# Ecogenomics/CheckM

Hardware: AMD Instinct MI355X
Metric: bins/hour (lineage_wf-equiv marker path: tree pass + analyze pass + qa, from genes.faa files) + residues*HMMs/s (higher is better)
Workload: dtype f16/i16 (SSV/MSV bytes held exactly, Viterbi words) + f32 (Forward/Backward)

## Files before the change

checkm_amd/csrc/cascade_dev.h:

```cpp
#pragma once
#include <hip/hip_runtime.h>
#include "dev_types.h"

namespace ckm {

constexpr float LOG2E_F = 1.44269504088896341f, LN2_F = 0.69314718055994529f;

__device__ __forceinline__ uint32_t queue_len(const WorkQueue &q) { return min(*q.count, q.cap); }

__device__ __forceinline__ float approx_ln(float x) { return __log2f(x) * LN2_F; }

__device__ __forceinline__ bool ws_alloc(const CascadeDev &cd, unsigned long long n, unsigned long long &off) {
  n = (n + 31ull) & ~31ull;
  off = atomicAdd(cd.ws_top, n);
  if (off + n > cd.ws_cap) { atomicOr(&cd.gcnt[CC_STATUS], (uint32_t)CS_WS); return false; }
  return true;
}

__device__ __forceinline__ bool ws2_alloc(const CascadeDev &cd, unsigned long long n, unsigned long long &off) {
  n = (n + 31ull) & ~31ull;
  const unsigned long long at = atomicAdd(cd.ws2_top, n);
  if (at + n > cd.ws2_cap) return false;
  off = cd.ws2_base + at;
  return true;
}

__device__ __forceinline__ void queue_push(const CascadeDev &cd, uint32_t *lists, int counter, int cls, uint32_t cap, uint32_t value, uint32_t overflow_bit) {
  const uint32_t pos = atomicAdd(&cd.cnt[counter + cls], 1u);
  if (pos < cap) lists[(size_t)cls * cap + pos] = value; else atomicOr(&cd.gcnt[CC_STATUS], overflow_bit);
}

__device__ __forceinline__ void pass_to_forward(const CascadeDev &cd, const DevModel &md, uint32_t pi, uint32_t model, uint32_t seq) {
  const int L = cd.seq_len[seq];
  unsigned long long off;
  if (!ws_alloc(cd, (unsigned long long)(L + 1) * 6ull, off)) return;
  const uint32_t t = atomicAdd(&cd.gcnt[CC_FWORK], 1u);
  if (t >= cd.cap_fwork) { atomicOr(&cd.gcnt[CC_STATUS], (uint32_t)CS_FWORK); return; }
  FbWork w;
  w.model = model; w.seq = seq; w.i0 = 0; w.Ld = L; w.Lcfg = L; w.multihit = 1;
  w.xs_off = off; w.aux_off = 0; w.mxf_off = 0; w.mxb_off = 0; w.path_off = 0;
  w.slot = t; w.full = 0; w.cand = pi; w.pass = 0xffffffffu;
  cd.fwork[t] = w;
  queue_push(cd, cd.fq, CC_FQ, md.fb_cls, cd.cap_fq, t, (uint32_t)CS_FWORK);
}

}
```

checkm_amd/csrc/cascade_regions.h:

```cpp
#pragma once
#include <hip/hip_runtime.h>
#include "dev_types.h"
#include "cascade_dev.h"
#include "xlane.h"

namespace ckm {

#ifndef CKM_LD2
#define CKM_LD2(p) __hip_atomic_load((p), __ATOMIC_RELAXED, __HIP_MEMORY_SCOPE_AGENT)
#endif

constexpr float RT1_F = 0.25f, RT2_F = 0.10f, RT3_F = 0.20f;
constexpr int ENS_CAP0 = 16;

__device__ __forceinline__ unsigned long long al32(unsigned long long v) { return (v + 31ull) & ~31ull; }

__device__ __forceinline__ void emit_region(const CascadeDev &cd, const DevModel &md, const FbWork &pw, int L, int ri, int rj, bool multi) {
  const uint32_t rid = atomicAdd(&cd.gcnt[CC_REG], 1u);
  if (rid >= cd.cap_reg) { atomicOr(&cd.gcnt[CC_STATUS], (uint32_t)CS_REG); return; }
  RegionRec rec; rec.pass = pw.pass; rec.i = ri; rec.j = rj; rec.multi = multi ? 1 : 0; rec.target = 0xffffffffu; rec.pad = 0;
  const unsigned long long Mp = (unsigned long long)md.fbQ * 64ull, Ld = (unsigned long long)(rj - ri + 1);
  unsigned long long off;
  if (!multi) {
    unsigned long long pos = 0;
    const unsigned long long xs = pos; pos = al32(pos + (Ld + 1) * 6);
    const unsigned long long aux = pos; pos = al32(al32(pos + (Ld + 1) * 3) + (Ld + 1) * 5);
    const unsigned long long mf = pos; pos = al32(pos + (Ld + 1) * 3 * Mp);
    unsigned long long mb = mf;
    if (!cd.env_inplace) { mb = pos; pos = al32(pos + (Ld + 1) * 2 * Mp); }
    if (!ws2_alloc(cd, pos, off)) rec.target = REGION_DEFERRED;
    else {
      const uint32_t e = atomicAdd(&cd.gcnt[CC_EWORK], 1u);
      if (e < cd.cap_ework) {
        FbWork w;
        w.model = pw.model; w.seq = pw.seq; w.i0 = ri - 1; w.Ld = (int32_t)Ld; w.Lcfg = L; w.multihit = 0;
        w.xs_off = off + xs; w.aux_off = off + aux; w.mxf_off = off + mf; w.mxb_off = off + mb; w.path_off = 0;
        w.slot = e; w.full = 1; w.cand = pw.cand; w.pass = pw.pass;
        cd.ework[e] = w;
        queue_push(cd, cd.eq, CC_EQ, md.fb_cls, cd.cap_eq, e, (uint32_t)CS_EWORK);
        rec.target = e;
      } else atomicOr(&cd.gcnt[CC_STATUS], (uint32_t)CS_EWORK);
    }
  } else {
    const unsigned long long cap = Ld < (unsigned long long)ENS_CAP0 ? Ld : (unsigned long long)ENS_CAP0;
    unsigned long long pos = 0;
    const unsigned long long nseg = pos; pos += 256;
    const unsigned long long seg = pos; pos += (unsigned long long)ENS_NSAMPLES * cap * 4;
    const unsigned long long n2 = pos; pos = al32(pos + Ld);
    const unsigned long long nres = pos;
    const unsigned long long xs = pos; pos = al32(pos + (Ld + 1) * 6);
    const unsigned long long mx = pos; pos = al32(pos + (Ld + 1) * 4 * Mp);
    const unsigned long long code = pos; pos = al32(pos + ((unsigned long long)ENS_NSAMPLES * (Ld + 1) + 1) / 2);
    const unsigned long long ratio = pos; pos = al32(pos + (unsigned long long)ENS_NSAMPLES * (Ld + 1));
    if (!ws2_alloc(cd, pos, off)) rec.target = REGION_DEFERRED;
    else {
      const uint32_t r = atomicAdd(&cd.gcnt[CC_RWORK], 1u);
      if (r < cd.cap_rwork) {
        EnsWork e;
        e.model = pw.model; e.seq = pw.seq; e.i0 = ri - 1; e.Ld = (int32_t)Ld; e.Lcfg = L; e.cap = (int32_t)cap;
        e.xs_off = off + xs; e.mx_off = off + mx; e.code_off = off + code; e.ratio_off = off + ratio;
        e.seg_off = off + seg; e.nseg_off = off + nseg; e.n2_off = off + n2;
        const unsigned long long hoff = atomicAdd(cd.hens_top, nres);
        e.host_off = (hoff + nres <= cd.hens_cap) ? hoff : ~0ull;
        if (e.host_off == ~0ull) atomicOr(&cd.gcnt[CC_STATUS], (uint32_t)CS_RWORK);
        rec.pad = (e.host_off == ~0ull) ? 0xffffffffu : (uint32_t)hoff;
        cd.ens[r] = e;
        FbWork w;
        w.model = pw.model; w.seq = pw.seq; w.i0 = ri - 1; w.Ld = (int32_t)Ld; w.Lcfg = L; w.multihit = 1;
        w.xs_off = e.xs_off; w.aux_off = 0; w.mxf_off = e.mx_off; w.mxb_off = 0; w.path_off = 0;
        w.slot = r; w.full = 2; w.cand = pw.cand; w.pass = pw.pass;
        cd.rwork[r] = w;
        queue_push(cd, cd.rq, CC_RQ, md.fb_cls, cd.cap_rq, r, (uint32_t)CS_RWORK);
        if (cd.ensq) { const uint32_t k = atomicAdd(cd.ensq_cnt, 1u); if (k < cd.cap_rwork) cd.ensq[k] = r; }
        rec.target = r;
      } else atomicOr(&cd.gcnt[CC_STATUS], (uint32_t)CS_RWORK);
    }
  }
  cd.h_reg[rid] = rec;
}

template <bool XL>
__device__ __forceinline__ void region_scan(const CascadeDev &cd, const DevModel &md, const FbWork &w, float *__restrict__ ws, int lane) {
  const int L = w.Ld;
  float *aux = ws + w.aux_off;
  float btp = 0.f, etp = 0.f;
  int ri = -1; bool trig = false;
  for (int base = 1; base <= L; base += 64) {
    const int row = base + lane;
    const bool ok = row <= L;
    const float bt = ok ? (XL ? CKM_LD2(&aux[(size_t)row * 3]) : aux[(size_t)row * 3]) : 0.f, et = ok ? (XL ? CKM_LD2(&aux[(size_t)row * 3 + 1]) : aux[(size_t)row * 3 + 1]) : 0.f,
                nj = ok ? (XL ? CKM_LD2(&aux[(size_t)row * 3 + 2]) : aux[(size_t)row * 3 + 2]) : 0.f;
    const int nrow = min(64, L - base + 1);
    const float btp0 = btp, etp0 = etp;
    float pb = 0.f, pe = 0.f;
    for (int r = 0; r < nrow; ++r) {
      btp = btp + read_lane(bt, r); etp = etp + read_lane(et, r);
      if (lane == r) { pb = btp; pe = etp; }
    }
    if (ok) { aux[(size_t)row * 3] = pb; aux[(size_t)row * 3 + 1] = pe; }
    __threadfence();
    __builtin_amdgcn_wave_barrier();
    float pbm = btp0, pem = etp0;
    for (int r = 0; r < nrow; ++r) {
      const float btn = read_lane(pb, r), etn = read_lane(pe, r), mo = 1.0f - read_lane(nj, r);
      const int j = base + r;
      if (!trig) {
        if (mo - (btn - pbm) < RT2_F) ri = j; else if (ri == -1) ri = j;
        if (mo >= RT1_F) trig = true;
      } else if (mo - (etn - pem) < RT2_F) {
        const float e0 = (ri - 1 >= 1) ? CKM_LD2(&aux[(size_t)(ri - 1) * 3 + 1]) : 0.f;
        float mx = -1.0f;
        for (int z = ri + lane; z <= j; z += 64) {
          const float bz = (z - 1 >= 1) ? CKM_LD2(&aux[(size_t)(z - 1) * 3]) : 0.f;
          const float a = CKM_LD2(&aux[(size_t)z * 3 + 1]) - e0, b = btn - bz;
          const float en = a < b ? a : b;
          if (en > mx) mx = en;
        }
        mx = wave_max(mx);
        if (lane == 0) emit_region(cd, md, w, L, ri, j, mx >= RT3_F);
        ri = -1; trig = false;
      }
      pbm = btn; pem = etn;
    }
  }
}

}
```

checkm_amd/csrc/ckm_api.hip:

```cpp
#include "ckm_host.h"

namespace ckm {
static thread_local std::string g_err;
void set_last_error(const std::string &m) { g_err = m; }

}

std::atomic<uint64_t> g_uid{1};

const std::string &ckm_seq_name(const ckm_seqs *s, uint32_t i) { return s->names.at(i); }
int ckm_ctx_device(const ckm_ctx *ctx) { return ctx->device; }
void ckm_ctx_parallel_for(ckm_ctx *ctx, size_t n, size_t chunk, const std::function<void(size_t, size_t)> &f) {
  if (ctx->w[0].pool) ctx->w[0].pool->run(n, chunk, f); else if (n) f(0, n);
}
void *ckm_ctx_reduce_scratch(ckm_ctx *ctx, size_t bytes) { ctx->reduce_scratch.ensure(bytes); return ctx->reduce_scratch.p; }

extern "C" const char *ckm_last_error(void) { return g_err.c_str(); }
extern "C" int ckm_abi_version(void) { return CKM_ABI_VERSION; }

extern "C" int ckm_device_count(int *n) {
  return guarded([&] {
    if (!n) throw Error(CKM_EINVAL, "n is NULL");
    int c = 0;
    hipError_t e = hipGetDeviceCount(&c);
    if (e != hipSuccess) { *n = 0; throw Error(CKM_ENODEV, std::string("hipGetDeviceCount: ") + hipGetErrorString(e)); }
    *n = c;
  });
}

extern "C" int ckm_ctx_create(int device, ckm_ctx **out) {
  setenv("GPU_MAX_HW_QUEUES", "16", 0);
  return guarded([&] {
    if (!out) throw Error(CKM_EINVAL, "out is NULL");
    *out = nullptr;
    int c = 0;
    if (hipGetDeviceCount(&c) != hipSuccess || c <= 0) throw Error(CKM_ENODEV, "no HIP device visible: libcheckm_hip has no CPU path");
    if (device < 0 || device >= c) throw Error(CKM_ENODEV, "device index out of range");
    HIPCHK(hipSetDevice(device));
    hipDeviceProp_t prop;
    HIPCHK(hipGetDeviceProperties(&prop, device));
    if (std::string(prop.gcnArchName).compare(0, 6, "gfx950") != 0)
      throw Error(CKM_ENODEV, std::string("device is ") + prop.gcnArchName + "; this library carries gfx950 code objects only");
    std::unique_ptr<ckm_ctx> ctx(new ckm_ctx());
    ctx->device = device;
    memset(&ctx->stats, 0, sizeof(ctx->stats));
    if (const char *e = getenv("CKM_WORKERS")) ctx->nclasses = std::max(1, std::min(NWORKERS, atoi(e)));
    ctx->nworkers = ctx->nclasses * ctx->ngroups;
    const int hw = (int)std::thread::hardware_concurrency();
    int host_threads = std::max(1, std::min(hw, std::max(8, std::min(16, hw / 8))));
    if (const char *e = getenv("CKM_HOST_THREADS")) host_threads = std::max(1, std::min(64, atoi(e)));
    size_t fre = 0, tot = 0;
    size_t budget = (size_t)8 << 30;
    if (hipMemGetInfo(&fre, &tot) == hipSuccess) budget = std::min<size_t>((size_t)96 << 30, fre / 4) / ctx->nworkers;
    if (const char *e = getenv("CKM_WS_BUDGET_MB")) budget = std::max<size_t>(16, strtoull(e, nullptr, 10)) << 20;
    const bool pooled = ctx->nworkers == 1;
    const int nside = choose_side_streams(ctx->nworkers);
    const int slot = pooled ? pool_next_slot(device) : 0;
    for (auto &w : ctx->w) {
      w.device = device; w.id = (int)(&w - ctx->w);
      if (&w - ctx->w >= ctx->nworkers) continue;
      if (pooled) pool_assign_streams(w, device, slot);
      else {
        w.own_streams = true;
        HIPCHK(hipStreamCreateWithFlags(&w.stream, hipStreamNonBlocking));
        w.nside = nside;
        w.nss = nside >= 8 ? 4 : std::max(1, nside / 3); w.nch = nside - w.nss;
        for (int k = 0; k < 16; ++k) {
          if (k >= nside) { w.side[k] = w.side[k % nside]; continue; }
          HIPCHK(hipStreamCreateWithFlags(&w.side[k], hipStreamNonBlocking));
        }
        HIPCHK(hipStreamCreateWithFlags(&w.ens_stream, hipStreamNonBlocking));
      }
      {
        int lo = 0, hi = 0;
        HIPCHK(hipDeviceGetStreamPriorityRange(&lo, &hi));
        HIPCHK(hipStreamCreateWithPriority(&w.late[0], hipStreamNonBlocking, hi));
        for (int k = 1; k < 4; ++k) w.late[k] = w.late[0];
      }
      for (auto &e : w.ev) HIPCHK(hipEventCreate(&e));
      for (auto &e : w.cev) HIPCHK(hipEventCreateWithFlags(&e, hipEventDisableTiming));
      for (auto &e : w.cls_ev) HIPCHK(hipEventCreateWithFlags(&e, hipEventDisableTiming));
      for (auto &e : w.grp_ev) HIPCHK(hipEventCreateWithFlags(&e, hipEventDisableTiming));
      for (auto &e : w.ens_ev) HIPCHK(hipEventCreateWithFlags(&e, hipEventDisableTiming));
      memset(&w.stats, 0, sizeof(w.stats));
      w.ws_budget = budget;
      if (!(getenv("CKM_WS_VMM") && atoi(getenv("CKM_WS_VMM")) == 0)) { w.ws.vmm = true; w.ws.va_bytes = budget + ((size_t)8 << 30); }
      if (const char *e = getenv("CKM_WS_PER_CELL")) w.caps.ws_per_cell = (float)atof(e);
      w.pool.reset(new HostPool(host_threads));
    }
    *out = ctx.release();
  });
}

extern "C" int ckm_ctx_reserve(ckm_ctx *ctx, uint64_t pairs, double cells) {
  return guarded([&] {
    if (!ctx) throw Error(CKM_EINVAL, "ctx is NULL");
    ctx->settle();
    Worker &w = ctx->w[0];
    const uint64_t est = (uint64_t)(1.05 * cells * (double)w.caps.ws_per_cell + (double)pairs * 24.0) + ((uint64_t)256 << 20);
    const size_t want = (size_t)std::min<uint64_t>(std::max<uint64_t>(est, (uint64_t)1 << 30), (uint64_t)w.ws_budget);
    if (w.ws.cap >= want) return;
    const int device = ctx->device;
    std::lock_guard<std::mutex> lock(ctx->reserve_mutex);
    ctx->reserve_thread = std::thread([&w, want, device] {
      if (hipSetDevice(device) != hipSuccess) return;
      try { w.ws.ensure(want); } catch (...) {  }
    });
  });
}

extern "C" void ckm_ctx_destroy(ckm_ctx *ctx) {
  if (!ctx) return;
  ctx->settle();
  (void)hipSetDevice(ctx->device);
  (void)hipDeviceSynchronize();
  for (auto &w : ctx->w) {
    if (!w.stream) continue;
    for (auto &e : w.ev) (void)hipEventDestroy(e);
    for (auto &e : w.cev) if (e) (void)hipEventDestroy(e);
    for (auto &e : w.cls_ev) if (e) (void)hipEventDestroy(e);
    for (auto &e : w.grp_ev) if (e) (void)hipEventDestroy(e);
    for (auto &e : w.ens_ev) if (e) (void)hipEventDestroy(e);
    if (w.late[0]) (void)hipStreamDestroy(w.late[0]);
    if (!w.own_streams) continue;
    for (int k = 0; k < w.nside; ++k) (void)hipStreamDestroy(w.side[k]);
    if (w.ens_stream) (void)hipStreamDestroy(w.ens_stream);
    (void)hipStreamDestroy(w.stream);
  }
  const int device = ctx->device;
  delete ctx;
  dev_cache_trim(device);
}

namespace {
struct Arena {
  std::vector<uint8_t> host;
  template <class T> size_t add(const std::vector<T> &v) {
    const size_t off = (host.size() + 255) & ~(size_t)255;
    host.resize(off + std::max<size_t>(16, v.size() * sizeof(T)));
    if (!v.empty()) memcpy(host.data() + off, v.data(), v.size() * sizeof(T));
    return off;
  }
};
}

extern "C" int ckm_profiles_load(ckm_ctx *ctx, const char *hmm_path, ckm_profiles **out) {
  return guarded([&] {
    if (!ctx || !hmm_path || !out) throw Error(CKM_EINVAL, "NULL argument");
    *out = nullptr;
    HIPCHK(hipSetDevice(ctx->device));
    std::unique_ptr<ckm_profiles> p(new ckm_profiles());
    p->ctx = ctx;
    p->hmm = read_hmm_file(hmm_path);
    const size_t n = p->hmm.size();
    p->prof.resize(n);
    p->too_long.assign(n, 0);
    {
      std::vector<std::unique_ptr<Error>> errs(n);
      auto one = [&](size_t lo, size_t hi) {
        for (size_t i = lo; i < hi; ++i) {
          try { p->prof[i] = configure_profile(p->hmm[i]); }
          catch (const Error &e) {
            if (e.code == CKM_ERANGE) { p->too_long[i] = 1; p->prof[i] = HostProfile(); p->prof[i].M = p->hmm[i].M; p->prof[i].ssvQ = p->prof[i].fbQ = p->prof[i].vitQH = 1; }
            else errs[i].reset(new Error(e));
          }
        }
      };
      if (ctx->w[0].pool && n > 8) ctx->w[0].pool->run(n, 4, one); else one(0, n);
      for (size_t i = 0; i < n; ++i) if (errs[i]) throw Error(*errs[i]);
    }
    Arena ar;
    struct Off { size_t ssv, ssvh, rbv, vit_e, vit_t, rf, ftr, v16e, v16t, ssv8; };
    std::vector<Off> off(n);
    for (size_t i = 0; i < n; ++i) {
      const HostProfile &hp = p->prof[i];
      off[i] = Off{ar.add(hp.ssv_tbl), ar.add(hp.ssv_tbl_h), ar.add(hp.rbv), ar.add(hp.vit_e), ar.add(hp.vit_t), ar.add(hp.rf), ar.add(hp.ftr), ar.add(hp.vit16_e), ar.add(hp.vit16_t), ar.add(hp.ssv8_tbl_h)};
    }
    std::unique_ptr<DevBuf> tables(new DevBuf());
    tables->ensure(std::max<size_t>(256, ar.host.size()));
    HIPCHK(hipMemcpy(tables->p, ar.host.data(), ar.host.size(), hipMemcpyHostToDevice));
    const uint8_t *base = tables->as<uint8_t>();
    p->tables.push_back(std::move(tables));
    for (size_t i = 0; i < n; ++i) {
      const HostHMM &h = p->hmm[i];
      const HostProfile &hp = p->prof[i];
      DevModel d;
      memset(&d, 0, sizeof(d));
      d.M = hp.M; d.ssvQ = hp.ssvQ; d.fbQ = hp.fbQ; d.vitQH = hp.vitQH;
      d.fb_cls = fb_class_id(hp.fbQ); d.vitx_cls = vit_class_id(hp.vitQH); d.vit16Q = hp.vit16Q;
      d.vit_cls = hp.vit16Q ? vit16_class_id(hp.vit16Q) : d.vitx_cls;
      if (!p->too_long[i] && (d.fb_cls < 0 || d.vit_cls < 0)) throw Error(CKM_ERANGE, "model " + h.name + " is longer than the instantiated kernel classes (DESIGN.md limits)");
      d.base_b = hp.base_b; d.bias_b = hp.bias_b; d.tbm_b = hp.tbm_b; d.tec_b = hp.tec_b; d.scale_b = hp.scale_b;
      d.scale_w = hp.scale_w; d.base_w = hp.base_w; d.wE_loop = hp.wE_loop; d.wE_move = hp.wE_move;
      d.fE_loop = hp.fE_loop; d.fE_move = hp.fE_move;
      d.bt00 = hp.bt00; d.bt01 = hp.bt01; d.bt10 = hp.bt10; d.bt11 = hp.bt11; d.bpi0 = hp.bpi0; d.bpi1 = hp.bpi1;
      for (int x = 0; x < NROWS; ++x) d.beo1[x] = hp.beo1[x];
      d.thr_msv_f1 = hp.thr_msv_f1; d.thr_msv_f1_nat = hp.thr_msv_f1_nat; d.thr_msv_f2 = hp.thr_msv_f2; d.thr_vit_f2 = hp.thr_vit_f2; d.thr_fwd_f3 = hp.thr_fwd_f3;
      d.ssv_tbl = reinterpret_cast<const int16_t *>(base + off[i].ssv); d.ssv_tbl_h = reinterpret_cast<const uint16_t *>(base + off[i].ssvh);
      d.rbv = base + off[i].rbv; d.vit_e = reinterpret_cast<const uint32_t *>(base + off[i].vit_e);
      d.vit_t = reinterpret_cast<const uint32_t *>(base + off[i].vit_t); d.rf = reinterpret_cast<const float *>(base + off[i].rf);
      d.ftr = reinterpret_cast<const float *>(base + off[i].ftr);
      d.ssv8_tbl_h = hp.ssv8Q ? reinterpret_cast<const uint16_t *>(base + off[i].ssv8) : nullptr;
      d.vit16_e = reinterpret_cast<const uint32_t *>(base + off[i].v16e); d.vit16_t = reinterpret_cast<const uint32_t *>(base + off[i].v16t);
      p->dm.push_back(d);
      if (!p->too_long[i]) p->maxMp = std::max(p->maxMp, hp.fbQ * NL);
    }
    p->d_models.ensure(p->dm.size() * sizeof(DevModel));
    HIPCHK(hipMemcpy(p->d_models.p, p->dm.data(), p->dm.size() * sizeof(DevModel), hipMemcpyHostToDevice));
    *out = p.release();
  });
}

extern "C" int ckm_profiles_count(const ckm_profiles *p, int32_t *n) {
  if (!p || !n) { set_last_error("NULL argument"); return CKM_EINVAL; }
  *n = (int32_t)p->hmm.size();
  return CKM_OK;
}

extern "C" int ckm_profiles_header(const ckm_profiles *p, int32_t i, ckm_model_header *o) {
  if (!p || !o || i < 0 || i >= (int32_t)p->hmm.size()) { set_last_error("bad argument"); return CKM_EINVAL; }
  const HostHMM &h = p->hmm[i];
  o->name = h.name.c_str(); o->acc = h.has_acc ? h.acc.c_str() : nullptr; o->desc = h.has_desc ? h.desc.c_str() : nullptr;
  o->leng = h.M; o->has_ga = h.has_ga; o->has_tc = h.has_tc; o->has_nc = h.has_nc;
  for (int k = 0; k < 2; ++k) { o->ga[k] = h.ga[k]; o->tc[k] = h.tc[k]; o->nc[k] = h.nc[k]; }
  for (int k = 0; k < 6; ++k) o->evparam[k] = h.evparam[k];
  o->searchable = p->too_long[(size_t)i] ? 0 : 1;
  return CKM_OK;
}

extern "C" void ckm_profiles_free(ckm_profiles *p) {
  if (!p) return;
  if (p->ctx) (void)hipSetDevice(p->ctx->device);
  delete p;
}

static void build_lentab(ckm_seqs *s) {
  HostProfile dummy;
  dummy.scale_b = (float)(3.0 / 0.69314718055994529);
  dummy.scale_w = (float)(500.0 / 0.69314718055994529);
  s->lentab.resize((size_t)s->maxL + 1);
  for (int L = 0; L <= s->maxL; ++L) {
    const LenCfg m = len_config(dummy, L, true), u = len_config(dummy, L, false);
    LenEntry e;
    e.loop_m = m.loop; e.move_m = m.move; e.loop_u = u.loop; e.move_u = u.move;
    e.nullsc = m.nullsc; e.bias_tail = m.bias_tail; e.w_move = m.w_move; e.tjb_b = m.tjb_b;
    s->lentab[L] = e;
  }
}

static SeqColumns seq_columns(ckm_seqs *s) {
  return SeqColumns{&s->bin_off, &s->seq_bin, &s->order, &s->order_off, &s->len, &s->off, &s->bin_res, &s->dsq, &s->names, &s->descs, &s->total_res, &s->maxL};
}

static void finish_seqs(ckm_seqs *s) {
  const uint32_t nseq = s->nseq;
  build_seq_order(ingest_threads(), seq_columns(s));
  build_lentab(s);
  hipStream_t up = s->ctx->w[0].late[3];
  trace_pt(&s->ctx->w[0], "seqs: tables built");
  s->d_res.ensure(s->dsq.size() + 16); s->d_off.ensure((size_t)nseq * 8 + 16); s->d_len.ensure((size_t)nseq * 4 + 16);
  s->d_order.ensure(s->order.size() * 4 + 16); s->d_lentab.ensure(s->lentab.size() * sizeof(LenEntry) + 16);
  trace_pt(&s->ctx->w[0], "seqs: device buffers allocated");
  {
    std::lock_guard<std::mutex> lock(s->ctx->upload_mutex);
    struct Part { DevBuf *d; const void *src; size_t bytes; };
    const Part parts[5] = {{&s->d_res, s->dsq.data(), s->dsq.size()}, {&s->d_off, s->off.data(), (size_t)nseq * 8}, {&s->d_len, s->len.data(), (size_t)nseq * 4},
                           {&s->d_order, s->order.data(), s->order.size() * 4}, {&s->d_lentab, s->lentab.data(), s->lentab.size() * sizeof(LenEntry)}};
    size_t tot = 0;
    for (auto &pt : parts) tot += (pt.bytes + 255) & ~(size_t)255;
    s->ctx->upload.begin(tot);
    for (auto &pt : parts) s->ctx->upload.put(up, pt.d->p, pt.src, pt.bytes);
    HIPCHK(hipStreamSynchronize(up));
  }
  trace_pt(&s->ctx->w[0], "seqs: uploaded");
// ... 259 lines not shown
```

checkm_amd/csrc/ckm_debug.hip:

```cpp
#include "ckm_host.h"

extern "C" int ckm_debug_stages(ckm_ctx *ctx_, const ckm_profiles *p, const ckm_seqs *s, const uint32_t *model, const uint32_t *seq,
                                uint32_t npairs, ckm_stage_scores *out) {
  return guarded([&] {
    if (!ctx_ || !p || !s || !model || !seq || !out) throw Error(CKM_EINVAL, "NULL argument");
    for (uint32_t j = 0; j < npairs; ++j) if (model[j] < p->hmm.size() && p->too_long[model[j]]) throw Error(CKM_ERANGE, "model longer than the instantiated kernel classes");
    ctx_->settle();
    Worker *ctx = &ctx_->w[0];
    ctx->plan_key.clear();
    HIPCHK(hipSetDevice(ctx->device));
    const DevModel *dm = p->d_models.as<DevModel>();
    const LenEntry *lt = s->d_lentab.as<LenEntry>();
    const uint8_t *res = s->d_res.as<uint8_t>();
    const uint64_t *off = s->d_off.as<uint64_t>();
    const int32_t *dlen = s->d_len.as<int32_t>();
    memset(out, 0, sizeof(*out) * npairs);
    std::vector<SsvBlockWork> work(npairs); std::vector<uint32_t> ids(seq, seq + npairs);
    std::map<int, std::vector<uint32_t>> byQ;
    for (uint32_t i = 0; i < npairs; ++i) {
      if (model[i] >= p->hmm.size() || seq[i] >= s->nseq) throw Error(CKM_EINVAL, "pair index out of range");
      work[i].model = model[i]; work[i].list_start = i; work[i].count = 1; work[i].pair_start = i; byQ[ssv_class(p->prof[model[i]])].push_back(i);
    }
    std::vector<SsvBlockWork> sorted; std::vector<std::pair<int, std::pair<size_t, size_t>>> groups;
    for (auto &kv : byQ) { groups.push_back({kv.first, {sorted.size(), kv.second.size()}}); for (uint32_t i : kv.second) sorted.push_back(work[i]); }
// ... 50 lines not shown
    std::vector<int32_t> vx(npairs); std::vector<float> vs(npairs);
    HIPCHK(hipMemcpyAsync(vx.data(), ctx->vitx.p, npairs * 4, hipMemcpyDeviceToHost, ctx->stream));
    HIPCHK(hipMemcpyAsync(vs.data(), ctx->vits.p, npairs * 4, hipMemcpyDeviceToHost, ctx->stream));
    HIPCHK(hipStreamSynchronize(ctx->stream));
    FbBatch fb; uint64_t pos = 0;
    for (uint32_t i = 0; i < npairs; ++i) {
      const int L = s->len[seq[i]];
      FbWork w; memset(&w, 0, sizeof(w));
      w.model = model[i]; w.seq = seq[i]; w.i0 = 0; w.Ld = L; w.Lcfg = L; w.multihit = 1; w.full = 0; w.slot = i;
      w.xs_off = pos; pos += ((uint64_t)(L + 1) * 6 + 31) & ~(uint64_t)31;
      w.aux_off = pos; pos += ((uint64_t)(L + 1) * 3 + 31) & ~(uint64_t)31;
      fb.work.push_back(w);
    }
    ctx->ws.ensure(pos * 4 + 256);
    run_fb(ctx, p, s, fb, true, false, false, nullptr);
    EventIndex ei; ei.build(fb.events, npairs);
    for (uint32_t i = 0; i < npairs; ++i) {
      const int L = s->len[seq[i]];
      const LenEntry &le = s->lentab[L];
      ckm_stage_scores &o = out[i];
      o.ssv_maxv = maxv[i]; o.msv_xJ = xJ[i]; o.msv_sc = usc[i]; o.null_sc = le.nullsc;
      o.msvp_xJ = xJp[i]; o.msvp_sc = uscp[i];
      const float p1 = (float)L / (float)(L + 1);
      const float nullsc = (float)(log((double)raw[(size_t)i * 3]) + (double)raw[(size_t)i * 3 + 1] * kLn2);
      o.bias_sc = nullsc + (float)L * logf(p1) + logf(1.0f - p1);
      o.vit_xC = vx[i]; o.vit_sc = vs[i];
      o.fwd_xC = fb.fout[i].xC; o.fwd_nscale = fb.fout[i].nscale;
      o.fwd_sc = finish_forward(fb.fout[i].xC, le.move_m, ei.scales(i));
    }
  });
}

extern "C" int ckm_debug_ssv(ckm_ctx *ctx_, const ckm_profiles *p, const ckm_seqs *s, uint32_t model, const uint32_t *seq, uint32_t n,
                             uint32_t per_block, int32_t lanes, uint16_t *smax, uint8_t *route, float *usc, int32_t *info) {
  return guarded([&] {
    if (!ctx_ || !p || !s || !seq || !smax || !route || !usc) throw Error(CKM_EINVAL, "NULL argument");
    if (model >= p->hmm.size()) throw Error(CKM_EINVAL, "model index out of range");
    if (p->too_long[model]) throw Error(CKM_ERANGE, "model longer than the instantiated kernel classes");
    if (n == 0 || n > (1u << 24)) throw Error(CKM_EINVAL, "between 1 and 2^24 sequences");
    if (lanes != 0 && lanes != 8 && lanes != 16) throw Error(CKM_EINVAL, "lanes must be 0, 8 or 16");
    std::vector<int64_t> pos_of(s->nseq, -1);
    for (uint32_t i = 0; i < n; ++i) {
      if (seq[i] >= s->nseq) throw Error(CKM_EINVAL, "sequence index out of range");
      if (s->len[seq[i]] <= 0) throw Error(CKM_EINVAL, "empty sequence (the lists of a search hold none)");
      if (pos_of[seq[i]] >= 0) throw Error(CKM_EINVAL, "sequence listed twice");
      pos_of[seq[i]] = i;
    }
    const HostProfile &hp = p->prof[model];
    int cls = ssv_class(hp);
    if (lanes == 8) { if (!hp.ssv8Q) throw Error(CKM_ERANGE, "the model has no 8-lane SSV image"); cls = 100 + hp.ssv8Q; }
    if (lanes == 16) { if (hp.ssvQ > 64) throw Error(CKM_ERANGE, "the model has no 16-lane SSV image"); cls = hp.ssvQ; }
    const uint32_t pb = per_block ? per_block : ssv_per_block(cls);
    const int threads = ssv_threads_for(cls);
    std::vector<SsvBlockWork> work;
    for (uint32_t a = 0; a < n; a += pb) { SsvBlockWork w; w.model = model; w.list_start = a; w.count = std::min(pb, n - a); w.pair_start = a; work.push_back(w); }
    if (info) { info[0] = cls; info[1] = threads; info[2] = (int32_t)pb; info[3] = (int32_t)work.size(); }
    ctx_->settle();
    Worker *ctx = &ctx_->w[0];
    ctx->plan_key.clear();
    HIPCHK(hipSetDevice(ctx->device));
    const DevModel *dm = p->d_models.as<DevModel>();
    const LenEntry *lt = s->d_lentab.as<LenEntry>();
    const uint8_t *res = s->d_res.as<uint8_t>();
    const uint64_t *off = s->d_off.as<uint64_t>();
    const int32_t *dlen = s->d_len.as<int32_t>();
    ctx->work.ensure(work.size() * sizeof(SsvBlockWork)); ctx->idx.ensure((size_t)n * 4); ctx->maxv.ensure((size_t)n * 2 + 64);
    ctx->surv.ensure((size_t)n * sizeof(PairRec)); ctx->nores.ensure((size_t)n * sizeof(PairRec)); ctx->counters.ensure(64);
    wcopy(ctx, ctx->work.p, work.data(), work.size() * sizeof(SsvBlockWork), hipMemcpyHostToDevice);
    wcopy(ctx, ctx->idx.p, seq, (size_t)n * 4, hipMemcpyHostToDevice);
    HIPCHK(hipMemsetAsync(ctx->maxv.p, 0xff, (size_t)n * 2, ctx->stream));
    HIPCHK(hipMemsetAsync(ctx->counters.p, 0, 64, ctx->stream));
    SsvEpi epi; memset(&epi, 0, sizeof(epi));
    epi.lentab = lt; epi.maxv = ctx->maxv.as<uint16_t>();
    if (launch_ssv(cls, (int)work.size(), threads, ctx->stream, ctx->work.as<SsvBlockWork>(), dm, res, off, dlen, ctx->idx.as<uint32_t>(), epi))
      throw Error(CKM_ERANGE, "no SSV kernel instance");
    const SsvEpi fin{lt, ctx->surv.as<PairRec>(), ctx->counters.as<uint32_t>(), n, ctx->nores.as<PairRec>(), ctx->counters.as<uint32_t>() + 1, n, nullptr};
    if (launch_ssv(cls, (int)work.size(), threads, ctx->stream, ctx->work.as<SsvBlockWork>(), dm, res, off, dlen, ctx->idx.as<uint32_t>(), fin))
      throw Error(CKM_ERANGE, "no SSV kernel instance");
    HIPCHK(hipGetLastError());
    uint32_t cnt[2] = {0, 0};
    HIPCHK(hipMemcpyAsync(smax, ctx->maxv.p, (size_t)n * 2, hipMemcpyDeviceToHost, ctx->stream));
    HIPCHK(hipMemcpyAsync(cnt, ctx->counters.p, 8, hipMemcpyDeviceToHost, ctx->stream));
    HIPCHK(hipStreamSynchronize(ctx->stream));
    if (cnt[0] > n || cnt[1] > n) throw Error(CKM_EHIP, "the SSV finish appended " + std::to_string(cnt[0]) + " survivors and " + std::to_string(cnt[1]) + " exact-kernel pairs for " + std::to_string(n) + " pairs");
    std::vector<PairRec> sv(cnt[0]), nr(cnt[1]);
    if (cnt[0]) wcopy(ctx, sv.data(), ctx->surv.p, (size_t)cnt[0] * sizeof(PairRec), hipMemcpyDeviceToHost);
    if (cnt[1]) wcopy(ctx, nr.data(), ctx->nores.p, (size_t)cnt[1] * sizeof(PairRec), hipMemcpyDeviceToHost);
    for (uint32_t i = 0; i < n; ++i) {
      if (smax[i] == 0xffffu) throw Error(CKM_EHIP, "the SSV kernel wrote no Smax for list entry " + std::to_string(i));
      route[i] = 0; usc[i] = 0.f;
    }
    auto place = [&](const PairRec &r, uint8_t code) {
      if (r.model != model || r.seq >= s->nseq || pos_of[r.seq] < 0) throw Error(CKM_EHIP, "the SSV finish reported a pair that was not listed: model " + std::to_string(r.model) + ", sequence " + std::to_string(r.seq));
      const size_t i = (size_t)pos_of[r.seq];
      if (route[i] != 0) throw Error(CKM_EHIP, "the SSV finish reported list entry " + std::to_string(i) + " twice");
      route[i] = code; usc[i] = r.usc;
    };
    for (const PairRec &r : sv) place(r, 1);
    for (const PairRec &r : nr) place(r, 2);
  });
}

extern "C" int ckm_debug_filters(ckm_ctx *ctx_, const ckm_profiles *p, const ckm_seqs *s, const uint32_t *model, const uint32_t *seq,
                                 const float *usc, const float *filtersc, uint32_t n, int32_t mode, uint32_t nblocks,
                                 ckm_filter_result *out, uint32_t *status) {
  return guarded([&] {
    if (!ctx_ || !p || !s || !model || !seq || !usc || !out || !status) throw Error(CKM_EINVAL, "NULL argument");
    if (mode < CKM_FILTERS_VIT16 || mode > CKM_FILTERS_CHAIN) throw Error(CKM_EINVAL, "unknown mode");
    if (mode != CKM_FILTERS_CHAIN && !filtersc) throw Error(CKM_EINVAL, "NULL argument");
    if (n == 0 || n > (1u << 22)) throw Error(CKM_EINVAL, "between 1 and 2^22 pairs");
    if (nblocks > 65536) throw Error(CKM_EINVAL, "at most 65536 workgroups");
    const uint32_t nb = nblocks ? nblocks : GRID_VIT;
    bool present[NVC] = {false};
    std::vector<std::vector<uint32_t>> vq(NVC);
    unsigned long long ws_need = 0;
    int q16 = -1;
    for (uint32_t i = 0; i < n; ++i) {
      if (model[i] >= p->hmm.size() || seq[i] >= s->nseq) throw Error(CKM_EINVAL, "pair index out of range");
      if (p->too_long[model[i]]) throw Error(CKM_ERANGE, "model longer than the instantiated kernel classes");
      if (s->len[seq[i]] <= 0) throw Error(CKM_EINVAL, "empty sequence (the lists of a search hold none)");
      const DevModel &d = p->dm[model[i]];
      if (mode == CKM_FILTERS_VIT16) {
        if (!d.vit16Q) throw Error(CKM_ERANGE, "the model has no 16-lane Viterbi image");
        if (q16 >= 0 && q16 != d.vit16Q) throw Error(CKM_EINVAL, "the pairs of a VIT16 call must share one 16-lane class");
        q16 = d.vit16Q;
      }
      const int c = (mode == CKM_FILTERS_VIT16 || mode == CKM_FILTERS_CHAIN) ? d.vit_cls : d.vitx_cls;
      if (c < 0 || c >= NVC || d.vitx_cls < NV16 || d.vitx_cls >= NVC || d.fb_cls < 0 || d.fb_cls >= NFC) throw Error(CKM_ERANGE, "no kernel instance for this model length");
      present[c] = true; present[d.vitx_cls] = true;
      if (mode != CKM_FILTERS_CHAIN) vq[c].push_back(i);
      ws_need += (((unsigned long long)(s->len[seq[i]] + 1) * 6ull) + 31ull) & ~31ull;
    }
    ctx_->settle();
    Worker *ctx = &ctx_->w[0];
    ctx->plan_key.clear();
    HIPCHK(hipSetDevice(ctx->device));
    const DevModel *dm = p->d_models.as<DevModel>();
    const LenEntry *lt = s->d_lentab.as<LenEntry>();
    const uint8_t *res = s->d_res.as<uint8_t>();
    const uint64_t *off = s->d_off.as<uint64_t>();
    const int32_t *dlen = s->d_len.as<int32_t>();
    hipStream_t st = ctx->stream;
    auto table = [](DevBuf &b, size_t bytes) { b.ensure(std::max<size_t>(64, bytes)); return b.p; };
    uint32_t *d_cnt = (uint32_t *)table(ctx->c_cnt, 2 * CC_SIZE * 4);
    unsigned long long *d_tops = (unsigned long long *)table(ctx->c_tops, 4 * 8);
    CascadeDev cd; memset(&cd, 0, sizeof(cd));
    cd.cand = (PairRec *)table(ctx->c_cand, (size_t)n * sizeof(PairRec)); cd.cap_cand = n;
    cd.bias_raw = (float *)table(ctx->c_bias, (size_t)n * 8);
    cd.vit_fast = (float *)table(ctx->c_vfast, (size_t)n * 4); cd.vit_exact = (float *)table(ctx->c_vexact, (size_t)n * 4);
    cd.vit_flag = (uint32_t *)table(ctx->c_vflag, (size_t)n * 4); cd.route = (uint8_t *)table(ctx->c_route, n);
    cd.vq = (uint32_t *)table(ctx->c_vq, (size_t)n * NVC * 4); cd.vxq = (uint32_t *)table(ctx->c_vxq, (size_t)n * NVC * 4); cd.cap_vq = n;
    cd.fq = (uint32_t *)table(ctx->c_fq, (size_t)n * NFC * 4); cd.cap_fq = n;
    cd.fwork = (FbWork *)table(ctx->c_fwork, (size_t)n * sizeof(FbWork)); cd.cap_fwork = n;
    cd.gcnt = d_cnt; cd.cnt = d_cnt + CC_SIZE;
    cd.ws_top = d_tops; cd.ws_cap = 2 * ws_need;
    cd.seq_len = dlen;
    cd.margin_msv = kMarginMsv; cd.margin_vit = kMarginVit; cd.margin_fwd = kMarginFwd;
    int32_t *d_xC = (int32_t *)table(ctx->vitx, (size_t)n * 4); float *d_sc = (float *)table(ctx->vits, (size_t)n * 4); uint32_t *d_flag = (uint32_t *)table(ctx->vitf, (size_t)n * 4);
    std::vector<PairRec> pr(n);
    for (uint32_t i = 0; i < n; ++i) { pr[i].model = model[i]; pr[i].seq = seq[i]; pr[i].usc = usc[i]; pr[i].filtersc = mode == CKM_FILTERS_CHAIN ? 0.f : filtersc[i]; }
    std::vector<uint32_t> cnt(2 * CC_SIZE, 0u);
    cnt[CC_SIZE + CC_CAND] = n;
    wcopy(ctx, cd.cand, pr.data(), (size_t)n * sizeof(PairRec), hipMemcpyHostToDevice);
    for (int c = 0; c < NVC; ++c) if (!vq[c].empty()) {
      cnt[CC_SIZE + CC_VQ + c] = (uint32_t)vq[c].size();
      wcopy(ctx, cd.vq + (size_t)c * n, vq[c].data(), vq[c].size() * 4, hipMemcpyHostToDevice);
    }
    wcopy(ctx, d_cnt, cnt.data(), cnt.size() * 4, hipMemcpyHostToDevice);
    HIPCHK(hipMemsetAsync(d_tops, 0, 4 * 8, st));
    auto sentinels = [&] {
      HIPCHK(hipMemsetAsync(cd.vit_fast, 0xff, (size_t)n * 4, st)); HIPCHK(hipMemsetAsync(cd.vit_exact, 0xff, (size_t)n * 4, st));
      HIPCHK(hipMemsetAsync(cd.vit_flag, 0xff, (size_t)n * 4, st));
    };
    sentinels();
    HIPCHK(hipMemsetAsync(cd.bias_raw, 0xff, (size_t)n * 8, st));
    HIPCHK(hipMemsetAsync(cd.route, mode == CKM_FILTERS_CHAIN ? 0xee : 1, n, st));
    HIPCHK(hipMemsetAsync(d_xC, 0xff, (size_t)n * 4, st)); HIPCHK(hipMemsetAsync(d_sc, 0xff, (size_t)n * 4, st)); HIPCHK(hipMemsetAsync(d_flag, 0xff, (size_t)n * 4, st));
    uint32_t *gc = cd.cnt;
    int rc = 0;
    auto exact_launches = [&] {
      for (int c = NVC - 1; c >= NV16; --c) if (present[c])
        rc |= launch_vit(kVitQH[c - NV16], std::max(64u, GRID_VIT / 4), st, WorkQueue{cd.vxq + (size_t)c * cd.cap_vq, gc + CC_VXQ + c, cd.cap_vq}, cd.cand, dm, lt, res, off, dlen, nullptr, nullptr, nullptr, false, &cd);
    };
    if (mode == CKM_FILTERS_CHAIN) {
      launch_bias_filter(st, GRID_MSV, cd, dm, lt, res, off);
      sentinels();
    }
    if (mode == CKM_FILTERS_WAVE_FAST_PLAIN) {
      for (int c = NVC - 1; c >= NV16; --c) if (present[c])
        rc |= launch_vit(kVitQH[c - NV16], nb, st, WorkQueue{cd.vq + (size_t)c * cd.cap_vq, gc + CC_VQ + c, cd.cap_vq}, cd.cand, dm, lt, res, off, dlen, d_xC, d_sc, d_flag, true, nullptr);
    } else {
      for (int c = NVC - 1; c >= 0; --c) if (present[c]) {
        const WorkQueue qv{cd.vq + (size_t)c * cd.cap_vq, gc + CC_VQ + c, cd.cap_vq};
        if (c < NV16) rc |= launch_vit16(kVit16Q[c], nb, st, qv, cd.cand, dm, lt, res, off, dlen, cd);
        else rc |= launch_vit(kVitQH[c - NV16], nb, st, qv, cd.cand, dm, lt, res, off, dlen, nullptr, nullptr, nullptr, true, &cd);
      }
      exact_launches();
    }
    if (rc) throw Error(CKM_ERANGE, "no Viterbi kernel instance");
    HIPCHK(hipGetLastError());
    std::vector<float> raw((size_t)n * 2), vfast(n), vexact(n), psc(n);
    std::vector<uint32_t> vflag(n), pflag(n), lists_vq((size_t)n * NVC), lists_vxq((size_t)n * NVC);
    std::vector<int32_t> pxC(n); std::vector<uint8_t> route(n);
    HIPCHK(hipMemcpyAsync(cnt.data(), d_cnt, cnt.size() * 4, hipMemcpyDeviceToHost, st));
    HIPCHK(hipMemcpyAsync(pr.data(), cd.cand, (size_t)n * sizeof(PairRec), hipMemcpyDeviceToHost, st));
    HIPCHK(hipMemcpyAsync(raw.data(), cd.bias_raw, (size_t)n * 8, hipMemcpyDeviceToHost, st));
    HIPCHK(hipMemcpyAsync(vfast.data(), cd.vit_fast, (size_t)n * 4, hipMemcpyDeviceToHost, st));
    HIPCHK(hipMemcpyAsync(vexact.data(), cd.vit_exact, (size_t)n * 4, hipMemcpyDeviceToHost, st));
    HIPCHK(hipMemcpyAsync(vflag.data(), cd.vit_flag, (size_t)n * 4, hipMemcpyDeviceToHost, st));
    HIPCHK(hipMemcpyAsync(route.data(), cd.route, n, hipMemcpyDeviceToHost, st));
    HIPCHK(hipMemcpyAsync(lists_vq.data(), cd.vq, (size_t)n * NVC * 4, hipMemcpyDeviceToHost, st));
    HIPCHK(hipMemcpyAsync(lists_vxq.data(), cd.vxq, (size_t)n * NVC * 4, hipMemcpyDeviceToHost, st));
    HIPCHK(hipMemcpyAsync(pxC.data(), d_xC, (size_t)n * 4, hipMemcpyDeviceToHost, st));
    HIPCHK(hipMemcpyAsync(psc.data(), d_sc, (size_t)n * 4, hipMemcpyDeviceToHost, st));
    HIPCHK(hipMemcpyAsync(pflag.data(), d_flag, (size_t)n * 4, hipMemcpyDeviceToHost, st));
    HIPCHK(hipStreamSynchronize(st));
    *status = cnt[CC_STATUS];
    const uint32_t nfw = std::min(cnt[CC_FWORK], n);
    std::vector<FbWork> fw(nfw);
    if (nfw) wcopy(ctx, fw.data(), cd.fwork, (size_t)nfw * sizeof(FbWork), hipMemcpyDeviceToHost);
    auto bits_of = [](float f) { uint32_t u; memcpy(&u, &f, 4); return u; };
    auto name = [&](uint32_t i) { return "pair " + std::to_string(i) + " (model " + std::to_string(model[i]) + ", sequence " + std::to_string(seq[i]) + ", L = " + std::to_string(s->len[seq[i]]) + ")"; };
    const bool plain = mode == CKM_FILTERS_WAVE_FAST_PLAIN;
    for (uint32_t i = 0; i < n; ++i) {
      ckm_filter_result &o = out[i];
      o.bias_d = raw[2 * (size_t)i]; o.bias_e = raw[2 * (size_t)i + 1]; o.filtersc = pr[i].filtersc;
      o.vit_fast = plain ? psc[i] : vfast[i]; o.vit_exact = vexact[i]; o.vit_flag = plain ? pflag[i] : vflag[i];
      o.vit_xC = plain ? pxC[i] : INT32_MAX; o.route = route[i]; o.n_vq = o.n_vxq = o.n_fwork = 0;
      if (pr[i].model != model[i] || pr[i].seq != seq[i]) throw Error(CKM_EHIP, "the candidate record of " + name(i) + " was overwritten");
    }
    if (cnt[CC_SIZE + CC_CAND] != n) throw Error(CKM_EHIP, "the candidate counter changed");
    for (int c = 0; c < NVC; ++c) {
      const uint32_t nv = cnt[CC_SIZE + CC_VQ + c], nx = cnt[CC_SIZE + CC_VXQ + c];
      if (nv > n || nx > n) throw Error(CKM_EHIP, "queue of class " + std::to_string(c) + " holds " + std::to_string(nv) + " FAST and " + std::to_string(nx) + " exact entries for " + std::to_string(n) + " pairs");
      if ((nv || nx) && !present[c]) throw Error(CKM_EHIP, "entries in the queue of class " + std::to_string(c) + ", which no pair of the call has");
      for (uint32_t k = 0; k < nv; ++k) {
        const uint32_t i = lists_vq[(size_t)c * n + k];
        if (i >= n) throw Error(CKM_EHIP, "FAST queue of class " + std::to_string(c) + ", position " + std::to_string(k) + ": " + std::to_string(i) + " is no pair of the call");
        if (p->dm[model[i]].vit_cls != c && !(mode != CKM_FILTERS_CHAIN && p->dm[model[i]].vitx_cls == c)) throw Error(CKM_EHIP, name(i) + " sits in the FAST queue of class " + std::to_string(c));
        if (out[i].n_vq++) throw Error(CKM_EHIP, name(i) + " sits twice in the FAST queue of class " + std::to_string(c));
        if (bits_of(out[i].vit_fast) == 0xffffffffu || out[i].vit_flag == 0xffffffffu) throw Error(CKM_EHIP, "FAST queue of class " + std::to_string(c) + ", position " + std::to_string(k) + ": the kernel wrote nothing for " + name(i));
      }
      for (uint32_t k = 0; k < nx; ++k) {
        const uint32_t i = lists_vxq[(size_t)c * n + k];
        if (i >= n) throw Error(CKM_EHIP, "exact queue of class " + std::to_string(c) + ", position " + std::to_string(k) + ": " + std::to_string(i) + " is no pair of the call");
        if (p->dm[model[i]].vitx_cls != c) throw Error(CKM_EHIP, name(i) + " sits in the exact queue of class " + std::to_string(c));
        if (out[i].n_vxq++) throw Error(CKM_EHIP, name(i) + " sits twice in the exact queue of class " + std::to_string(c));
        if (bits_of(out[i].vit_exact) == 0xffffffffu) throw Error(CKM_EHIP, "exact queue of class " + std::to_string(c) + ", position " + std::to_string(k) + ": the kernel wrote nothing for " + name(i));
      }
    }
    if (cnt[CC_FWORK] > n) throw Error(CKM_EHIP, std::to_string(cnt[CC_FWORK]) + " Forward items for " + std::to_string(n) + " pairs");
    for (uint32_t t = 0; t < nfw; ++t) {
      const uint32_t i = fw[t].cand;
      if (i >= n || fw[t].model != model[i] || fw[t].seq != seq[i]) throw Error(CKM_EHIP, "Forward item " + std::to_string(t) + " is no pair of the call");
      if (out[i].n_fwork++) throw Error(CKM_EHIP, name(i) + " was handed to Forward twice");
    }
    if (mode == CKM_FILTERS_CHAIN) for (uint32_t i = 0; i < n; ++i) {
      if (out[i].route == 0xee || bits_of(out[i].bias_d) == 0xffffffffu) throw Error(CKM_EHIP, "the bias filter wrote nothing for " + name(i));
    }
  });
}

extern "C" int ckm_debug_envelopes(ckm_ctx *ctx_, const ckm_profiles *p, const ckm_seqs *s, const uint32_t *model, const uint32_t *seq,
                                   const int32_t *ienv, const int32_t *jenv, uint32_t n, ckm_envelope_result *out) {
  return guarded([&] {
    if (!ctx_ || !p || !s || !model || !seq || !ienv || !jenv || !out) throw Error(CKM_EINVAL, "NULL argument");
    ctx_->settle();
    Worker *ctx = &ctx_->w[0];
    HIPCHK(hipSetDevice(ctx->device));
    std::vector<EnvReq> req(n); std::vector<EnvRes> res;
    for (uint32_t i = 0; i < n; ++i) {
      if (model[i] >= p->hmm.size() || seq[i] >= s->nseq || ienv[i] < 1 || jenv[i] > s->len[seq[i]] || jenv[i] < ienv[i]) throw Error(CKM_EINVAL, "bad envelope");
      req[i] = {model[i], seq[i], ienv[i], jenv[i]};
    }
    rescore_envelopes(ctx, p, s, req, res);
    for (uint32_t i = 0; i < n; ++i) {
      out[i].envsc = res[i].envsc; out[i].oasc = res[i].oasc; out[i].fwd_xC = res[i].xC; out[i].nscale = res[i].nscale; out[i].ok = res[i].ok;
      for (int x = 0; x < 20; ++x) out[i].null2[x] = res[i].null2[x];
      out[i].hmm_from = res[i].hmm_from; out[i].hmm_to = res[i].hmm_to; out[i].ali_from = res[i].ali_from; out[i].ali_to = res[i].ali_to;
    }
  });
}

extern "C" int ckm_debug_region(ckm_ctx *ctx_, const ckm_profiles *p, const ckm_seqs *s, uint32_t model, uint32_t seq, int32_t ireg, int32_t jreg,
                                float *n2sum, int32_t *segs, int32_t *nseg, int32_t cap, int32_t *env, int32_t envcap, int32_t *nenv) {
  return guarded([&] {
    if (!ctx_ || !p || !s || !n2sum || !segs || !nseg || !env || !nenv) throw Error(CKM_EINVAL, "NULL argument");
    if (model >= p->hmm.size() || seq >= s->nseq || ireg < 1 || jreg > s->len[seq] || jreg < ireg) throw Error(CKM_EINVAL, "bad region");
    ctx_->settle();
    Worker *ctx = &ctx_->w[0];
    HIPCHK(hipSetDevice(ctx->device));
    std::vector<RegionReq> req{{model, seq, ireg, jreg}}; std::vector<RegionRes> res;
    run_ensembles(ctx, p, s, req, res);
    const RegionRes &r = res[0];
    for (size_t i = 0; i < r.n2sum.size(); ++i) n2sum[i] = r.n2sum[i];
    for (int t = 0; t < ENS_NSAMPLES; ++t) {
      if (r.nseg[t] > cap) throw Error(CKM_ERANGE, "segment table too small");
      nseg[t] = r.nseg[t];
      for (int d = 0; d < r.nseg[t]; ++d) { const Seg &g = r.segs[(size_t)t * r.cap + d]; int32_t *o = segs + ((size_t)t * cap + d) * 4; o[0] = g.sqfrom; o[1] = g.sqto; o[2] = g.hmmfrom; o[3] = g.hmmto; }
    }
    if ((int)r.env.size() > envcap) throw Error(CKM_ERANGE, "envelope table too small");
    *nenv = (int32_t)r.env.size();
    for (size_t e = 0; e < r.env.size(); ++e) { env[e * 4] = r.env[e].sqfrom; env[e * 4 + 1] = r.env[e].sqto; env[e * 4 + 2] = r.env[e].hmmfrom; env[e * 4 + 3] = r.env[e].hmmto; }
  });
}
```

checkm_amd/csrc/ckm_host.h:

```cpp
#pragma once
#include <hip/hip_runtime.h>
#include <algorithm>
#include <array>
#include <atomic>
#include <chrono>
#include <cmath>
#include <condition_variable>
#include <cstring>
#include <exception>
#include <functional>
#include <map>
#include <memory>
#include <mutex>
#include <numeric>
#include <thread>
#include "ckm_internal.h"
#include "dev_types.h"
#include "host_pool.h"
#include "stream_plan.h"

namespace ckm {

int launch_ssv(int Q, int nblocks, int threads, hipStream_t stream, const SsvBlockWork *work, const DevModel *models,
               const uint8_t *res, const uint64_t *seq_off, const int32_t *seq_len, const uint32_t *lists, const SsvEpi &epi );
void launch_msv_full(hipStream_t stream, uint32_t nblocks, WorkQueue queue, const PairRec *pairs, const DevModel *models, const LenEntry *lentab,
                     const uint8_t *res, const uint64_t *seq_off, const int32_t *seq_len, int32_t *out_xJ, float *out_usc, int maxMp,
                     const CascadeDev *cd );
void launch_bias(hipStream_t stream, PairRec *pairs, uint32_t npairs, const DevModel *models, const LenEntry *lentab,
                 const uint8_t *res, const uint64_t *seq_off, const int32_t *seq_len, float *raw);
int launch_msv16(int Q, uint32_t nblocks, hipStream_t stream, WorkQueue queue, const PairRec *pairs, const DevModel *models, const LenEntry *lentab,
                 const uint8_t *res, const uint64_t *seq_off, const int32_t *seq_len, const CascadeDev &cd, int32_t *out_xJ = nullptr , float *out_usc = nullptr);
int launch_vit16(int Q, uint32_t nblocks, hipStream_t stream, WorkQueue queue, const PairRec *pairs, const DevModel *models, const LenEntry *lentab,
                 const uint8_t *res, const uint64_t *seq_off, const int32_t *seq_len, const CascadeDev &cd);
int launch_vit(int QH, uint32_t nblocks, hipStream_t stream, WorkQueue queue, const PairRec *pairs, const DevModel *models,
               const LenEntry *lentab, const uint8_t *res, const uint64_t *seq_off, const int32_t *seq_len, int32_t *out_xC, float *out_sc,
               uint32_t *out_flag, bool fast, const CascadeDev *cd );
int launch_fwd(int Q, uint32_t nblocks, hipStream_t stream, WorkQueue queue, FbWork *work, const DevModel *models,
               const LenEntry *lentab, const uint8_t *res, const uint64_t *seq_off, float *ws, FwdOut *out,
               ScaleEvent *events, uint32_t *nevents, uint32_t cap_events, const CascadeDev *cd );
int launch_bwd(int Q, uint32_t nblocks, hipStream_t stream, WorkQueue queue, const FbWork *work, const DevModel *models,
               const LenEntry *lentab, const uint8_t *res, const uint64_t *seq_off, float *ws, const FwdOut *fout, int32_t *range_err);
int launch_oa(int Q, uint32_t nblocks, hipStream_t stream, WorkQueue queue, const FbWork *work, const DevModel *models,
              float *ws, const int32_t *range_err, const FwdOut *fout, EnvOut *out);

void launch_ensemble(hipStream_t stream, const EnsWork *work, const uint32_t *list , const uint32_t *count, uint32_t cap, uint32_t grid_regions, int max_Mp,
                     const DevModel *models, const LenEntry *lentab, const uint8_t *res, const uint64_t *seq_off, float *ws, const uint32_t *seeds,
                     float *host_res );
void launch_bias_filter(hipStream_t stream, uint32_t nblocks, const CascadeDev &cd, const DevModel *models, const LenEntry *lentab,
                        const uint8_t *res, const uint64_t *seq_off);
void launch_regions(hipStream_t stream, uint32_t nblocks, const uint32_t *list, const uint32_t *count, uint32_t cap, const FbWork *fwork,
                    const CascadeDev &cd, const DevModel *models, float *ws);
#define HIPCHK(expr)                                                                                         \
  do {                                                                                                       \
    hipError_t e_ = (expr);                                                                                  \
    if (e_ != hipSuccess) throw Error(CKM_EHIP, std::string(#expr) + ": " + hipGetErrorString(e_));          \
  } while (0)

struct DevCache {
  std::mutex m;
  std::multimap<size_t, void *> free_[16];
  size_t cached[16] = {0};
  static DevCache &get() { static DevCache c; return c; }
  void *take(int dev, size_t want, size_t &got) {
    std::lock_guard<std::mutex> lock(m);
    auto &f = free_[dev & 15];
    auto it = f.lower_bound(want);
    if (it != f.end() && it->first <= want + want / 2 + (1 << 20)) { void *p = it->second; got = it->first; cached[dev & 15] -= got; f.erase(it); return p; }
    return nullptr;
  }
  bool give(int dev, void *p, size_t cap) {
    if (cap >= ((size_t)2 << 30)) return false;
    std::lock_guard<std::mutex> lock(m);
    if (cached[dev & 15] + cap > ((size_t)64 << 30)) return false;
    free_[dev & 15].emplace(cap, p); cached[dev & 15] += cap;
    return true;
  }
  void trim(int dev) {
    std::multimap<size_t, void *> f;
    { std::lock_guard<std::mutex> lock(m); f.swap(free_[dev & 15]); cached[dev & 15] = 0; }
    for (auto &kv : f) (void)hipFree(kv.second);
  }
};
inline void dev_cache_trim(int dev) { DevCache::get().trim(dev); }

struct DevBuf {
  void *p = nullptr; size_t cap = 0; int dev = -1;
  bool vmm = false; size_t va_bytes = (size_t)128 << 30, chunk_bytes = 0; std::vector<hipMemGenericAllocationHandle_t> chunks;
  void drop(bool drained = false) {
    if (!p) return;
    if (!drained || dev < 0 || !DevCache::get().give(dev, p, cap)) (void)hipFree(p);
    p = nullptr; cap = 0;
  }
  void ensure(size_t bytes) {
    if (bytes <= cap) return;
    if (vmm) {
      if (p) { grow_mapped(bytes); return; }
      try { grow_mapped(bytes); return; }
      catch (const Error &) { if (p || cap) throw; vmm = false; }
    }
    drop();
    (void)hipGetDevice(&dev);
    size_t want = bytes + std::min<size_t>(bytes / 4, (size_t)1 << 30) + 256;
    size_t got = 0;
    if (void *q = DevCache::get().take(dev, want, got)) { p = q; cap = got; return; }
    hipError_t e = hipMalloc(&p, want);
    if (e != hipSuccess) {
      DevCache::get().trim(dev);
      e = hipMalloc(&p, want);
    }
    if (e != hipSuccess) { p = nullptr; throw Error(CKM_ENOMEM, "hipMalloc of " + std::to_string(want) + " bytes failed: " + hipGetErrorString(e)); }
    cap = want;
  }
  void grow_mapped(size_t bytes) {
    int dev = 0; (void)hipGetDevice(&dev);
    hipMemAllocationProp prop = {};
    prop.type = hipMemAllocationTypePinned; prop.location.type = hipMemLocationTypeDevice; prop.location.id = dev;
    auto fail = [&](const char *what, hipError_t e) { throw Error(CKM_ENOMEM, std::string(what) + " failed while growing a mapped buffer to " + std::to_string(bytes) + " bytes: " + hipGetErrorString(e)); };
    if (!p) {
      size_t gran = 0;
      hipError_t e = hipMemGetAllocationGranularity(&gran, &prop, hipMemAllocationGranularityRecommended);
      if (e != hipSuccess || !gran) fail("hipMemGetAllocationGranularity", e);
      chunk_bytes = (((size_t)1 << 30) + gran - 1) / gran * gran;
      va_bytes = (va_bytes + chunk_bytes - 1) / chunk_bytes * chunk_bytes;
      e = hipMemAddressReserve(&p, va_bytes, 0, nullptr, 0);
      if (e != hipSuccess) { p = nullptr; fail("hipMemAddressReserve", e); }
    }
    const size_t want = (bytes + 256 + chunk_bytes - 1) / chunk_bytes * chunk_bytes;
    if (want > va_bytes) throw Error(CKM_ENOMEM, "a mapped buffer cannot grow beyond its " + std::to_string(va_bytes) + " reserved bytes");
    hipMemAccessDesc acc = {}; acc.location.type = hipMemLocationTypeDevice; acc.location.id = dev; acc.flags = hipMemAccessFlagsProtReadWrite;
    while (cap < want) {
      hipMemGenericAllocationHandle_t h;
      hipError_t e = hipMemCreate(&h, chunk_bytes, &prop, 0);
      if (e != hipSuccess) { DevCache::get().trim(dev); e = hipMemCreate(&h, chunk_bytes, &prop, 0); }
      if (e != hipSuccess) fail("hipMemCreate", e);
      e = hipMemMap(static_cast<char *>(p) + cap, chunk_bytes, 0, h, 0);
      if (e != hipSuccess) { (void)hipMemRelease(h); fail("hipMemMap", e); }
      e = hipMemSetAccess(static_cast<char *>(p) + cap, chunk_bytes, &acc, 1);
      if (e != hipSuccess) { (void)hipMemUnmap(static_cast<char *>(p) + cap, chunk_bytes); (void)hipMemRelease(h); fail("hipMemSetAccess", e); }
      chunks.push_back(h); cap += chunk_bytes;
    }
  }
  template <class T> T *as() const { return reinterpret_cast<T *>(p); }
  ~DevBuf() {
    if (vmm) {
      if (p && cap) (void)hipMemUnmap(p, cap);
      for (auto h : chunks) (void)hipMemRelease(h);
      if (p) (void)hipMemAddressFree(p, va_bytes);
    } else drop(std::uncaught_exceptions() == 0);
  }
  DevBuf() = default; DevBuf(const DevBuf &) = delete; DevBuf &operator=(const DevBuf &) = delete;
};

struct PinnedBuf {
  void *p = nullptr; size_t cap = 0;
  void ensure(size_t bytes) {
    if (bytes <= cap) return;
    if (p) (void)hipHostFree(p);
    p = nullptr; cap = 0;
    const size_t want = bytes + bytes / 4 + 4096;
    if (hipHostMalloc(&p, want, hipHostMallocPortable | hipHostMallocMapped) != hipSuccess) { p = nullptr; throw Error(CKM_ENOMEM, "hipHostMalloc failed"); }
    cap = want;
  }
  template <class T> T *as() const { return reinterpret_cast<T *>(p); }
  ~PinnedBuf() { if (p) (void)hipHostFree(p); }
};


void launch_upload(hipStream_t st, void *dst, const void *src_pinned, size_t bytes);
struct Stager {
  static constexpr size_t HALF = (size_t)16 << 20;
  PinnedBuf buf; hipEvent_t ev[2] = {nullptr, nullptr}; bool busy[2] = {false, false}; int half = 0; size_t top = 0;
  void begin(size_t ) {
    if (!buf.p) { buf.ensure(2 * HALF); for (auto &e : ev) HIPCHK(hipEventCreateWithFlags(&e, hipEventDisableTiming)); }
    busy[0] = busy[1] = false; half = 0; top = 0;
  }
  void put(hipStream_t st, void *dst, const void *src, size_t bytes) {
    const uint8_t *from = static_cast<const uint8_t *>(src); uint8_t *to = static_cast<uint8_t *>(dst);
    while (bytes) {
      if (top == HALF) {
        HIPCHK(hipEventRecord(ev[half], st)); busy[half] = true;
        half ^= 1; top = 0;
        if (busy[half]) { HIPCHK(hipEventSynchronize(ev[half])); busy[half] = false; }
      }
      const size_t n = std::min(bytes, HALF - top);
      uint8_t *stage = buf.as<uint8_t>() + (size_t)half * HALF + top;
      memcpy(stage, from, n);
      launch_upload(st, to, stage, n);
      top = std::min(HALF, (top + n + 255) & ~(size_t)255);
      from += n; to += n; bytes -= n;
    }
  }
  ~Stager() { for (auto &e : ev) if (e) (void)hipEventDestroy(e); }
};

struct CallStream {
  hipStream_t st = nullptr;
  hipEvent_t ev[8] = {};
  bool own = false;
  void open(int device) {
    HIPCHK(hipSetDevice(device));
    HIPCHK(hipStreamCreateWithFlags(&st, hipStreamNonBlocking));
    own = true;
    for (auto &e : ev) HIPCHK(hipEventCreate(&e));
  }
  void borrow(hipStream_t s) {
    st = s;
    for (auto &e : ev) HIPCHK(hipEventCreate(&e));
  }
  void mark(int k) { HIPCHK(hipEventRecord(ev[k], st)); }
  float ms(int a, int b) { float t = 0.f; HIPCHK(hipEventElapsedTime(&t, ev[a], ev[b])); return t; }
  template <class F> void timed(double &acc, F &&fn) {
    mark(0);
    fn();
    mark(1);
    HIPCHK(hipEventSynchronize(ev[1]));
    acc += ms(0, 1);
  }
  ~CallStream() {
    for (auto &e : ev) if (e) (void)hipEventDestroy(e);
    if (own) { (void)hipStreamSynchronize(st); (void)hipStreamDestroy(st); }
  }
  CallStream() = default; CallStream(const CallStream &) = delete; CallStream &operator=(const CallStream &) = delete;
};

}

using namespace ckm;

extern std::atomic<uint64_t> g_uid;

struct Worker {
  int device = 0;
  int id = 0;
  hipStream_t stream = nullptr;
  hipStream_t ens_stream = nullptr;
  hipStream_t side[16];
  int nside = 0;
  int nss = 0, nch = 0;
  bool own_streams = false;
  hipEvent_t ev[8];
  ckm_search_stats stats;
  std::vector<uint64_t> plan_key;
  std::vector<std::pair<int, std::pair<size_t, size_t>>> plan_groups;
  uint64_t plan_npairs = 0, plan_nblocks = 0, plan_residue_hmm = 0, plan_cells = 0, plan_pairs = 0;
  PinnedBuf h_a, h_b, h_ens;
  DevBuf work, maxv, surv, nores, counters, cand, raw, idx, vitx, vits, vitf, fbwork, fbidx, fbmodel, ws, fout, events, rerr, envout, fullx, fullu, msvwork, msvlist, enswork, ensseeds, ws_ens, enscount, vitq;
  size_t ws_budget = (size_t)8 << 30;
  std::unique_ptr<HostPool> pool;
  struct CascadeCaps { uint32_t fwork = 0, ework = 0, rwork = 0, pass = 0, reg = 0, events_f = 0, events_e = 0, seen_rwork = 0; uint64_t hens = 0;
                       uint32_t div_cand = 12, div_nores = 48, div_fwork = 160, div_ework = 256, div_rwork = 32768;
                       uint32_t fl_cand = 4096, fl_nores = 2048, fl_fwork = 2048, fl_ework = 1024, fl_rwork = 256; float ws_per_cell = 11.f, z1_per_pair = 64.f; } caps;
  DevBuf c_cnt, c_cand, c_nores, c_bias, c_vfast, c_vexact, c_vflag, c_route, c_vq, c_vxq, c_fq, c_bq, c_eq, c_rq, c_fwork, c_ework, c_rwork, c_ens, c_ensq,
         c_fout_f, c_fout_e, c_fout_r, c_rerr_e, c_rerr_r, c_tops, c_events_r, c_pass, c_reg, c_hens, c_envout, c_events_f, c_events_e;
  PinnedBuf h_cnt, h_pass, h_reg, h_envout, h_events_f, h_events_e, h_hens, h_tops;
  hipEvent_t cev[4] = {nullptr, nullptr, nullptr, nullptr};
  hipEvent_t cls_ev[16] = {};
  bool ens_pending = false;
  hipEvent_t ens_ev[17] = {};
  PinnedBuf wstage; std::mutex wstage_mutex;
  Stager stager;
  hipStream_t late[4] = {};
  bool late_round = false;
  hipEvent_t grp_ev[192] = {};
};

constexpr int kVitQH[ckm::NVW] = {1, 2, 3, 4, 5, 6, 7, 8, 10, 12, 14, 16, 24, 32};
constexpr int kVit16Q[ckm::NV16] = {1, 2, 3, 4, 5, 6, 7, 8, 10, 12, 14, 16};
constexpr int kFbQ[ckm::NFC] = {1, 2, 3, 4, 6, 8, 12, 16, 24, 32, 48, 64};
constexpr int kSsvNone = 65;
inline int vit_class_id(int QH) { for (int i = 0; i < ckm::NVW; ++i) if (kVitQH[i] == QH) return ckm::NV16 + i; return -1; }
inline int vit16_class_id(int Q16) { for (int i = 0; i < ckm::NV16; ++i) if (kVit16Q[i] == Q16) return i; return -1; }
inline int fb_class_id(int Q) { for (int i = 0; i < ckm::NFC; ++i) if (kFbQ[i] == Q) return i; return -1; }

constexpr float kMarginMsv = 0.01f, kMarginVit = 0.01f, kMarginFwd = 0.05f;
constexpr uint32_t GRID_FB = 4096, GRID_VIT = 2048, GRID_MSV = 1024;

constexpr int NWORKERS = 8;

struct ckm_ctx {
  int device = 0;
  int nworkers = 1;
  int nclasses = 1, ngroups = 1;
  DevBuf reduce_scratch;
  Worker w[NWORKERS];
  ckm_search_stats stats;
  std::mutex ssv_mutex;
  std::condition_variable ssv_cv; int ssv_turn = 0;
  std::mutex upload_mutex; Stager upload;
  std::thread reserve_thread;
  std::string reserve_error;
  std::mutex reserve_mutex;
  void settle() { std::lock_guard<std::mutex> lock(reserve_mutex); if (reserve_thread.joinable()) reserve_thread.join(); }
  std::atomic<uint64_t> fallbacks{0};
  hipEvent_t ssv_prev_done = nullptr;
};

struct ckm_profiles {
  ckm_ctx *ctx = nullptr;
  uint64_t uid = g_uid++;
  std::vector<HostHMM> hmm;
  std::vector<HostProfile> prof;
  std::vector<DevModel> dm;
  DevBuf d_models;
  std::vector<std::unique_ptr<DevBuf>> tables;
  std::vector<uint8_t> too_long;
  int maxMp = 0;
};


struct ckm_seqs {
  ckm_ctx *ctx = nullptr;
  uint64_t uid = 0;
  uint32_t nseq = 0, nbins = 0;
  std::vector<uint32_t> bin_off, seq_bin;
  std::vector<int32_t> len;
  std::vector<uint64_t> off;
  std::vector<uint8_t> dsq;
  std::vector<std::string> names, descs;
  std::vector<LenEntry> lentab;
  DevBuf d_res, d_off, d_len, d_lentab;
  uint64_t total_res = 0;
  int maxL = 0;
  std::vector<uint32_t> order, order_off;
  std::vector<uint64_t> bin_res;
  DevBuf d_order;
};

struct ckm_hits {
  std::vector<uint64_t> bin_row_off;
  std::vector<uint32_t> seq, model;
  std::vector<int32_t> tlen, qlen, dom_idx, ndom, hmm_from, hmm_to, ali_from, ali_to, env_from, env_to;
  std::vector<double> full_evalue, c_evalue, i_evalue;
  std::vector<float> full_score, full_bias, dom_score, dom_bias, acc;
  uint32_t nbins = 0;
};

static inline void drain_after_error(int code) {
  if (code != CKM_EINVAL && code != CKM_ENODEV) (void)hipDeviceSynchronize();
}
template <class F>
static inline int guarded(F &&f) {
  try { f(); return CKM_OK; }
  catch (const Error &e) { set_last_error(e.what()); drain_after_error(e.code); return e.code; }
  catch (const std::bad_alloc &) { set_last_error("out of host memory"); drain_after_error(CKM_ENOMEM); return CKM_ENOMEM; }
  catch (const std::exception &e) { set_last_error(e.what()); return CKM_EINVAL; }
}

namespace ckm {

constexpr double kLn2 = 0.69314718055994529;
constexpr double kLog2R = 1.44269504088896341;
constexpr float kOmega = 1.0f / 256.0f;
constexpr float RT1 = 0.25f, RT2 = 0.10f, RT3 = 0.20f;

struct Domain {
  int ienv, jenv; float envsc, oasc, domcorrection; int hmm_from, hmm_to, ali_from, ali_to;
  float dombias, bitscore; double lnP; bool reported;
};
struct Hit {
  uint32_t model, seq; int L; float pre_score, score; double lnP; std::vector<Domain> dom; int nreported;
};
struct Cand {
  PairRec r; float fwdsc; float fwd_xC; uint32_t slot; bool alive;
};

struct EventIndex {
  std::vector<uint32_t> first;
  std::vector<std::pair<int, float>> ev;
  void build(const ScaleEvent *e, size_t n, size_t nslots) {
    first.assign(nslots + 1, 0);
    for (size_t k = 0; k < n; ++k) if (e[k].slot < nslots) first[e[k].slot + 1]++;
    for (size_t k = 0; k < nslots; ++k) first[k + 1] += first[k];
    ev.resize(first[nslots]);
    std::vector<uint32_t> at(first.begin(), first.end() - 1);
    for (size_t k = 0; k < n; ++k) if (e[k].slot < nslots) ev[at[e[k].slot]++] = {e[k].row, e[k].scale};
    for (size_t k = 0; k < nslots; ++k) if (first[k + 1] - first[k] > 1) std::sort(ev.begin() + first[k], ev.begin() + first[k + 1]);
  }
  void build(const std::vector<ScaleEvent> &v, size_t nslots) { build(v.data(), v.size(), nslots); }
  std::vector<float> scales(uint32_t slot) const { std::vector<float> r; for (uint32_t k = first[slot]; k < first[slot + 1]; ++k) r.push_back(ev[k].second); return r; }
};

struct FbBatch {
  std::vector<FbWork> work;
  std::vector<FwdOut> fout;
  std::vector<ScaleEvent> events;
  std::vector<int32_t> rerr;
  std::vector<EnvOut> envout;
};

struct EnvReq { uint32_t model, seq; int ienv, jenv; };

struct EnvRes { bool ok; float envsc, oasc, xC; int nscale; float null2[KP]; int hmm_from, hmm_to, ali_from, ali_to; };

struct Seg { int32_t sqfrom, sqto, hmmfrom, hmmto; };

struct RegionReq { uint32_t model, seq; int ireg, jreg; };

struct RegionRes {
  std::vector<float> n2sum;
  std::vector<Seg> segs;
  std::vector<int32_t> nseg;
  int cap = 0;
  std::vector<Seg> env;
};

void pool_run(Worker *w, size_t n, size_t chunk, const std::function<void(size_t, size_t)> &f);
void wcopy(Worker *w, void *dst, const void *src, size_t bytes, hipMemcpyKind kind);
double now_ms();
float bits(float sc, float nullsc);
float finish_forward(float xC, float move, const std::vector<float> &scales);
int ssv_threads_for(int Q);
int ssv_class(const HostProfile &hp);
uint32_t ssv_per_block(int cls);
int choose_side_streams(int nworkers);
int hw_queue_budget();
void pool_assign_streams(Worker &w, int device, int slot);
// ... 31 lines not shown
```

checkm_amd/csrc/ckm_search.hip:

```cpp
#include "ckm_host.h"

namespace {

#define CKM_TRACE_PT(label) trace_pt(ctx, label)

}


typedef std::map<std::pair<uint32_t, uint32_t>, std::vector<Hit>> HitMap;

void assemble_hits(Worker *ctx, const ckm_profiles *p, const ckm_seqs *s, DomStage &ds, HitMap &by_bin_model) {
  const std::vector<DomItem> &items = ds.items; const std::vector<RegionRes> &regres = ds.regres; const std::vector<EnvReq> &envreq = ds.envreq;
  const std::vector<int> &env_region = ds.env_region; std::vector<EnvRes> &envres = ds.envres; const std::vector<int> &nregions = ds.nregions;
  const std::vector<std::pair<size_t, size_t>> &env_of_pass = ds.env_of_pass;
  std::vector<std::pair<size_t, size_t>> items_of(ds.pass.size(), {0, 0});
  { size_t it = 0; for (size_t q = 0; q < ds.pass.size(); ++q) { items_of[q].first = it; while (it < items.size() && items[it].pass == q) ++it; items_of[q].second = it; } }
  std::vector<Hit> hit_of(ds.pass.size()); std::vector<uint8_t> has_hit(ds.pass.size(), 0);
  pool_run(ctx, ds.pass.size(), 32, [&](size_t qlo, size_t qhi) {
  std::vector<float> n2sc;
  for (size_t q = qlo; q < qhi; ++q) {
    const PassInfo &c = ds.pass[q];
    const HostHMM &hm = p->hmm[c.model];
    const int L = s->len[c.seq];
    const uint8_t *dsq = s->dsq.data() + s->off[c.seq];
// ... 410 lines not shown
    if (const char *e = getenv("CKM_STREAM_LAYOUT")) {
      int a = 0, b = 0, c = 0, d = 0;
      if (sp.plan.budget < 16 && sscanf(e, "%d,%d,%d,%d", &a, &b, &c, &d) == 4 && a >= 1 && a <= 4 && b >= 0 && b <= 10 && (c == 0 || c == 1) && d >= 0 &&
          d <= kPlanContexts && a + b + c + d <= sp.plan.budget)
        plan_layout(sp.plan, a, b, c, d);
    }
    std::vector<hipStream_t> h((size_t)sp.plan.nhandles, nullptr);
    for (auto &s : h) HIPCHK(hipStreamCreateWithFlags(&s, hipStreamNonBlocking));
    sp.h = std::move(h);
  }
  const StreamPlan &pl = sp.plan;
  const int c = slot % pl.contexts;
  w.own_streams = false;
  w.nss = pl.nss; w.nch = pl.nch; w.nside = pl.nss + pl.nch;
  w.stream = sp.h[(size_t)pl.main_h[c]];
  w.ens_stream = sp.h[(size_t)pl.ens_h[c]];
  for (int k = 0; k < 16; ++k) w.side[k] = sp.h[(size_t)pl.side_h[c][k < w.nside ? k : k % w.nside]];
}

static bool late_on() { static const bool on = !(getenv("CKM_LATE_PRIO") && atoi(getenv("CKM_LATE_PRIO")) == 0); return on; }
static bool baton_on() { static const bool on = !(getenv("CKM_SSV_BATON") && atoi(getenv("CKM_SSV_BATON")) == 0); return on; }

static int cascade_dev(Worker *ctx, ckm_ctx *owner, int my_turn, const ckm_profiles *p, const ckm_seqs *s, const SeqRange &rng,
                        const std::vector<uint32_t> &my_models, const std::vector<std::vector<uint32_t>> &model_bins, HitMap &by_bin_model) {
  HIPCHK(hipSetDevice(ctx->device));
  const double t_start = now_ms();
  ckm_search_stats &st = ctx->stats;
  memset(&st, 0, sizeof(st));
  const DevModel *dm = p->d_models.as<DevModel>();
  const LenEntry *lt = s->d_lentab.as<LenEntry>();
  const uint8_t *res = s->d_res.as<uint8_t>();
  const uint64_t *off = s->d_off.as<uint64_t>();
  const int32_t *dlen = s->d_len.as<int32_t>();
  bool took_turn = false;
  struct TurnGuard {
    ckm_ctx *o; int t; bool *took;
    ~TurnGuard() { if (*took) return; std::unique_lock<std::mutex> l(o->ssv_mutex); o->ssv_cv.wait(l, [&] { return o->ssv_turn == t; }); o->ssv_turn++; o->ssv_cv.notify_all(); }
  } turn_guard{owner, my_turn, &took_turn};

  uint64_t pair_budget = (uint64_t)1 << 29;
  if (const char *e = getenv("CKM_PAIR_BUDGET")) pair_budget = std::max<uint64_t>(1, strtoull(e, nullptr, 10));
  struct MW { uint32_t model; uint64_t pair_base; uint64_t npairs; };
  std::vector<MW> mws;
  uint64_t total_pairs = 0;
  for (uint32_t m1 : my_models) {
    uint64_t n = 0;
    for (uint32_t b : model_bins[m1]) n += rng.hi[b] - rng.lo[b];
    if (n == 0) continue;
    mws.push_back({m1, total_pairs, n}); total_pairs += n;
  }
  if (total_pairs == 0) { st.ms_total = now_ms() - t_start; return 0; }
  if (total_pairs > pair_budget) return 2;

  hipStream_t ms = ctx->stream;
  const uint32_t nbins = s->nbins;
  std::vector<std::vector<uint32_t>> cut(1, rng.lo);
  int nparts = 1, Lcut = 0;
  std::vector<int> Lcuts;
  {
    uint64_t split_min = 2000000;
    if (const char *e = getenv("CKM_SPLIT_MIN_PAIRS")) split_min = strtoull(e, nullptr, 10);
    std::vector<double> shares{0.25};
    if (const char *e = getenv("CKM_LONG_SHARE")) {
      shares.clear();
      for (const char *q = e; *q;) {
        char *end = nullptr;
        const double v = strtod(q, &end);
        if (end == q) break;
        if (v > 0.0 && v < 1.0) shares.push_back(v);
        if (*end != ',') break;
        q = end + 1;
      }
    }
    if (total_pairs >= split_min && !shares.empty()) {
      std::vector<uint64_t> by_len((size_t)s->maxL + 2, 0);
      uint64_t total = 0;
      for (uint32_t b = 0; b < nbins; ++b) for (uint32_t k = rng.lo[b]; k < rng.hi[b]; ++k) { const int L = s->len[s->order[k]]; by_len[L] += (uint64_t)L; total += (uint64_t)L; }
      uint64_t acc = 0; double want = 0.0; size_t si = 0;
      want = shares[0];
      for (int L = s->maxL; L >= 1 && si < shares.size(); --L) {
        acc += by_len[L];
        if ((double)acc >= want * (double)total) {
          if (L - 1 > 0 && (Lcuts.empty() || L - 1 < Lcuts.back())) Lcuts.push_back(L - 1);
          if (++si < shares.size()) want += shares[si];
        }
      }
      for (int lc : Lcuts) {
        std::vector<uint32_t> c(nbins);
        for (uint32_t b = 0; b < nbins; ++b) {
          uint32_t lo = rng.lo[b], hi = rng.hi[b];
          while (lo < hi) { const uint32_t m = (lo + hi) / 2; if (s->len[s->order[m]] > lc) lo = m + 1; else hi = m; }
          c[b] = lo;
        }
        cut.push_back(std::move(c));
      }
      nparts = (int)Lcuts.size() + 1;
      if (!Lcuts.empty()) Lcut = Lcuts[0];
    }
  }
  cut.push_back(rng.hi);
  auto enc = [](int cls) { return cls >= 100 ? cls - 100 : 40 + cls; };
  auto dec = [](int code) { return code < 40 ? 100 + code : code - 40; };
  std::vector<std::pair<int, std::pair<size_t, size_t>>> groups;
  {
    std::vector<uint64_t> key{p->uid, s->uid, pair_budget, (uint64_t)Lcut, rng.tag, 0xdeull};
    for (int lc : Lcuts) key.push_back(0xc0000000ull + (uint64_t)lc);
    for (auto &mw : mws) { key.push_back(0xffffffffull + mw.model); for (uint32_t b : model_bins[mw.model]) key.push_back(b); }
    if (key == ctx->plan_key) {
      groups = ctx->plan_groups;
      st.pairs_ssv += ctx->plan_pairs; st.residue_hmm += ctx->plan_residue_hmm; st.cells_ssv += ctx->plan_cells;
    } else {
      struct Run { uint32_t model, first, count; uint64_t pair0; };
      std::map<int, std::vector<Run>> runs;
      uint64_t c_pairs = 0, c_res = 0, c_cells = 0;
      for (auto &mw : mws) {
        const int Q = ssv_class(p->prof[mw.model]);
        uint64_t pb = mw.pair_base;
        for (uint32_t b : model_bins[mw.model]) {
          const uint32_t o0 = rng.lo[b], n = rng.hi[b] - o0;
          for (int part = 0; part < nparts; ++part) {
            const uint32_t a0 = cut[part][b] - o0, a1 = cut[part + 1][b] - o0;
            if (a1 > a0) runs[part * 1000 + enc(Q)].push_back({mw.model, o0 + a0, a1 - a0, pb + a0});
          }
          pb += n; c_res += rng.res[b]; c_cells += rng.res[b] * (uint64_t)p->prof[mw.model].M;
        }
        c_pairs += mw.npairs;
      }
      st.pairs_ssv += c_pairs; st.residue_hmm += c_res; st.cells_ssv += c_cells;
      std::vector<SsvBlockWork> allw;
      for (auto &kv : runs) {
        const int Q = dec(kv.first % 1000); const uint32_t per_block = ssv_per_block(Q);
        const size_t first = allw.size();
        std::vector<Run> &rv = kv.second;
        std::stable_sort(rv.begin(), rv.end(), [&](const Run &x, const Run &y) { return s->len[s->order[x.first]] > s->len[s->order[y.first]]; });
        for (uint32_t a = 0;; a += per_block) {
          bool any = false;
          for (const Run &r : rv) if (a < r.count) {
            any = true;
            SsvBlockWork w; w.model = r.model; w.list_start = r.first + a; w.count = std::min(per_block, r.count - a); w.pair_start = (uint32_t)(r.pair0 + a);
            allw.push_back(w);
          }
          if (!any) break;
        }
        groups.push_back({kv.first, {first, allw.size() - first}});
      }
      ctx->work.ensure(allw.size() * sizeof(SsvBlockWork));
      ctx->stager.begin(allw.size() * sizeof(SsvBlockWork));
      ctx->stager.put(ctx->late[2], ctx->work.p, allw.data(), allw.size() * sizeof(SsvBlockWork));
      HIPCHK(hipStreamSynchronize(ctx->late[2]));
      ctx->plan_key = key; ctx->plan_groups = groups; ctx->plan_nblocks = allw.size(); ctx->plan_pairs = c_pairs; ctx->plan_residue_hmm = c_res; ctx->plan_cells = c_cells;
    }
  }
  struct Sub { int Q; int maxM = 0; size_t first, nblocks; uint64_t pairs = 0; bool vit[NVC] = {false}, fb[NFC] = {false};
               uint32_t cap_cand = 0, cap_nores = 0, cap_f = 0, cap_e = 0, cap_r = 0; size_t o_cand = 0, o_nores = 0, o_vq = 0, o_f = 0, o_e = 0, o_r = 0; };
  std::vector<Sub> subs;
  {
    std::map<int, size_t> at;
    for (auto &g : groups) { Sub sb; sb.Q = dec(g.first % 1000); sb.first = g.second.first; sb.nblocks = g.second.second; at[g.first] = subs.size(); subs.push_back(sb); }
    for (auto &mw : mws) {
      for (int part = 0; part < nparts; ++part) {
        uint64_t np = 0;
        for (uint32_t b : model_bins[mw.model]) np += cut[part + 1][b] - cut[part][b];
        auto it = at.find(part * 1000 + enc(ssv_class(p->prof[mw.model])));
        if (it == at.end()) continue;
        Sub &sb = subs[it->second]; sb.pairs += np; sb.vit[p->dm[mw.model].vit_cls] = true; sb.vit[p->dm[mw.model].vitx_cls] = true; sb.fb[p->dm[mw.model].fb_cls] = true; sb.maxM = std::max(sb.maxM, p->prof[mw.model].M);
      }
    }
  }
  const size_t NG = subs.size();
  if (NG > 192) return 2;
  CKM_TRACE_PT("plan ready");

  Worker::CascadeCaps &cp = ctx->caps;
  size_t tot_cand = 0, tot_nores = 0, tot_f = 0, tot_e = 0, tot_r = 0;
  const uint64_t shrink = getenv("CKM_CAP_SHRINK") ? std::max(1, atoi(getenv("CKM_CAP_SHRINK"))) : 1;
  auto capof = [&](uint64_t pairs, uint32_t div, uint64_t floor_) {
    return (uint32_t)std::min<uint64_t>(std::max<uint64_t>(shrink > 1 ? 8 : floor_, pairs / ((uint64_t)div * shrink)), 0x7ffffff0ull); };
  for (Sub &sb : subs) {
    sb.cap_cand = capof(sb.pairs, cp.div_cand, cp.fl_cand);
    sb.cap_nores = sb.Q == kSsvNone ? (uint32_t)std::min<uint64_t>(sb.pairs + 64, 0x7ffffff0ull)
                                    : capof(sb.pairs, cp.div_nores, cp.fl_nores);
    sb.cap_f = capof(sb.pairs, cp.div_fwork, cp.fl_fwork);
    sb.cap_e = capof(sb.pairs, cp.div_ework, cp.fl_ework);
    sb.cap_r = capof(sb.pairs, cp.div_rwork, cp.fl_rwork);
    sb.o_cand = tot_cand; tot_cand += sb.cap_cand; sb.o_nores = tot_nores; tot_nores += sb.cap_nores;
    sb.o_vq = sb.o_cand * NVC;
    sb.o_f = tot_f * NFC; tot_f += sb.cap_f; sb.o_e = tot_e * NFC; tot_e += sb.cap_e; sb.o_r = tot_r * NFC; tot_r += sb.cap_r;
  }
  auto grow = [](uint32_t &v, uint64_t want) { if (v < want) v = (uint32_t)std::min<uint64_t>(want, 0xfffffff0ull); };
  grow(cp.fwork, tot_f); grow(cp.ework, tot_e); grow(cp.rwork, tot_r);
  grow(cp.pass, std::max<uint64_t>(1 << 13, tot_e)); grow(cp.reg, (uint64_t)cp.ework + cp.rwork);
  grow(cp.events_f, std::max<uint64_t>(1 << 18, (uint64_t)cp.fwork * 16));
  grow(cp.events_e, std::max<uint64_t>(1 << 16, (uint64_t)cp.ework * 16));
  cp.hens = std::max<uint64_t>(cp.hens, std::min<uint64_t>(cp.rwork, (uint64_t)4 * cp.seen_rwork + 8192) * (256 + ENS_NSAMPLES * 16 * 4 + 1024));
  double cell_sum = 0.0;
  {
    for (auto &mw : mws) { const double Mp = (double)(p->prof[mw.model].fbQ * NL); cell_sum += (double)model_bins[mw.model].size() * (Mp + 64.0) * Mp; }
    const uint64_t est = (uint64_t)(cell_sum * cp.ws_per_cell + (double)total_pairs * 24.0) + ((uint64_t)256 << 20);
    const size_t want = (size_t)std::min<uint64_t>(std::max<uint64_t>(est, (uint64_t)1 << 30), (uint64_t)ctx->ws_budget);
    if (ctx->ws.cap < want) ctx->ws.ensure(want);
  }
  const uint64_t ws_floats = ctx->ws.cap / 4;
  CKM_TRACE_PT("workspace ready");
  uint32_t *d_gcnt = dev_table<uint32_t>(ctx->c_cnt, (NG + 1) * CC_SIZE);
  unsigned long long *d_tops = dev_table<unsigned long long>(ctx->c_tops, 4);
  CascadeDev cd0; memset(&cd0, 0, sizeof(cd0));
  PairRec *d_cand = dev_table<PairRec>(ctx->c_cand, tot_cand), *d_nores = dev_table<PairRec>(ctx->c_nores, tot_nores);
  float *d_bias = dev_table<float>(ctx->c_bias, tot_cand * 2), *d_vfast = dev_table<float>(ctx->c_vfast, tot_cand), *d_vexact = dev_table<float>(ctx->c_vexact, tot_cand);
  uint32_t *d_vflag = dev_table<uint32_t>(ctx->c_vflag, tot_cand); uint8_t *d_route = dev_table<uint8_t>(ctx->c_route, tot_cand);
  uint32_t *d_vq = dev_table<uint32_t>(ctx->c_vq, tot_cand * NVC), *d_vxq = dev_table<uint32_t>(ctx->c_vxq, tot_cand * NVC);
  uint32_t *d_fq = dev_table<uint32_t>(ctx->c_fq, tot_f * NFC), *d_bq = dev_table<uint32_t>(ctx->c_bq, tot_f * NFC);
  uint32_t *d_eq = dev_table<uint32_t>(ctx->c_eq, tot_e * NFC), *d_rq = dev_table<uint32_t>(ctx->c_rq, tot_r * NFC);
  cd0.gcnt = d_gcnt;
  cd0.fwork = dev_table<FbWork>(ctx->c_fwork, cp.fwork); cd0.cap_fwork = cp.fwork;
  cd0.ework = dev_table<FbWork>(ctx->c_ework, cp.ework); cd0.cap_ework = cp.ework;
  cd0.rwork = dev_table<FbWork>(ctx->c_rwork, cp.rwork); cd0.ens = dev_table<EnsWork>(ctx->c_ens, cp.rwork); cd0.cap_rwork = cp.rwork;
  uint32_t *d_ensq = dev_table<uint32_t>(ctx->c_ensq, (size_t)4 * cp.rwork);
  {
    const uint64_t z1 = std::min<uint64_t>(ws_floats / 2, ((uint64_t)((double)total_pairs * cp.z1_per_pair) + ((uint64_t)64 << 20)) / 4) & ~(uint64_t)31;
    cd0.ws_top = d_tops; cd0.ws_cap = z1;
    cd0.ws2_top = d_tops + 2; cd0.ws2_base = z1; cd0.ws2_cap = ws_floats - z1;
  }
  cd0.h_pass = dev_table<PassRec>(ctx->c_pass, cp.pass); cd0.cap_pass = cp.pass;
  cd0.h_reg = dev_table<RegionRec>(ctx->c_reg, cp.reg); cd0.cap_reg = cp.reg;
  float *d_hens = dev_table<float>(ctx->c_hens, cp.hens);
  cd0.hens_top = d_tops + 1; cd0.hens_cap = cp.hens;
  cd0.seq_len = dlen;
  cd0.margin_msv = kMarginMsv; cd0.margin_vit = kMarginVit; cd0.margin_fwd = kMarginFwd;
  cd0.env_inplace = env_inplace() ? 1u : 0u;
  FwdOut *d_fout_f = dev_table<FwdOut>(ctx->c_fout_f, cp.fwork), *d_fout_e = dev_table<FwdOut>(ctx->c_fout_e, cp.ework), *d_fout_r = dev_table<FwdOut>(ctx->c_fout_r, cp.rwork);
  int32_t *d_rerr_e = dev_table<int32_t>(ctx->c_rerr_e, cp.ework);
  ScaleEvent *d_events_r = dev_table<ScaleEvent>(ctx->c_events_r, 1 << 16);
  EnvOut *d_envout = dev_table<EnvOut>(ctx->c_envout, cp.ework);
  ScaleEvent *d_events_f = dev_table<ScaleEvent>(ctx->c_events_f, cp.events_f), *d_events_e = dev_table<ScaleEvent>(ctx->c_events_e, cp.events_e);
  uint32_t *h_cnt = pin_table<uint32_t>(ctx->h_cnt, (NG + 1) * CC_SIZE);
  ensure_ens_seeds(ctx);
  float *ws = ctx->ws.as<float>();
  CKM_TRACE_PT("tables ready");
  const int NS = ctx->nside;
  const int NSS = ctx->nss;
  const int NCH = ctx->nch;

  {
    std::unique_lock<std::mutex> lock(owner->ssv_mutex);
    owner->ssv_cv.wait(lock, [&] { return owner->ssv_turn == my_turn; });
  }
  CKM_TRACE_PT("ssv turn taken");
  const int stop = getenv("CKM_CHAIN_STOP") ? atoi(getenv("CKM_CHAIN_STOP")) : 99;
  HIPCHK(hipMemsetAsync(d_gcnt, 0, (NG + 1) * CC_SIZE * sizeof(uint32_t), ms));
  HIPCHK(hipMemsetAsync(d_tops, 0, 4 * sizeof(unsigned long long), ms));
  if (owner->ssv_prev_done) HIPCHK(hipStreamWaitEvent(ms, owner->ssv_prev_done, 0));
  DeviceBaton &baton = device_baton(owner->device);
  struct InFlight { DeviceBaton &b; InFlight(DeviceBaton &x) : b(x) { b.searches++; } ~InFlight() { b.searches--; } } in_flight{baton};
  std::unique_lock<std::mutex> baton_lock(baton.m, std::defer_lock);
  if (baton_on()) {
    baton_lock.lock();
    if (!baton.ev[0]) for (auto &e : baton.ev) HIPCHK(hipEventCreateWithFlags(&e, hipEventDisableTiming));
    if (baton.recorded) HIPCHK(hipStreamWaitEvent(ms, baton.ev[baton.k], 0));
  }
  HIPCHK(hipEventRecord(ctx->ev[0], ms));
  HIPCHK(hipEventRecord(ctx->cev[0], ms));
  for (int k = 0; k < NS; ++k) HIPCHK(hipStreamWaitEvent(ctx->side[k], ctx->cev[0], 0));
  {
    std::vector<size_t> launch_order;
    {
      size_t g0 = 0;
      for (int part = 0; part < nparts; ++part) {
        size_t g1 = g0;
        while (g1 < NG && groups[g1].first / 1000 == part) ++g1;
        for (size_t g = g1; g-- > g0;) launch_order.push_back(g);
        g0 = g1;
      }
    }
    int ens_Mp = NL;
    for (const Sub &sb : subs) for (int c = 0; c < NFC; ++c) if (sb.fb[c]) ens_Mp = std::max(ens_Mp, kFbQ[c] * NL);
    hipStream_t es = ctx->ens_stream;
    bool ens_launched = false;
    auto ens_slot = [](int part) { return std::min(part, 3); };
    auto flush_part = [&](int part) {
      if (stop < 13) return;
      const int k0 = NCH > 0 ? NSS : 0, k1 = NCH > 0 ? NS : NSS;
      for (int k = k0; k < k1; ++k) { HIPCHK(hipEventRecord(ctx->ens_ev[k], ctx->side[k])); HIPCHK(hipStreamWaitEvent(es, ctx->ens_ev[k], 0)); }
      const int sl = ens_slot(part);
      launch_ensemble(es, cd0.ens, d_ensq + (size_t)sl * cp.rwork, d_gcnt + CC_ENSQ + sl, cp.rwork, 64, ens_Mp, dm, lt, res, off, ws, ctx->ensseeds.as<uint32_t>(), d_hens);
      ens_launched = true;
    };
    int gi = 0, cur_part = -1;
    for (size_t g : launch_order) {
      const int gi_now = gi++;
      const Sub &sb = subs[g];
      const int part = groups[g].first / 1000;
      if (cur_part >= 0 && ens_slot(part) != ens_slot(cur_part)) flush_part(cur_part);
      cur_part = part;
      hipStream_t sv = ctx->side[gi_now % NSS];
      CascadeDev cd = cd0;
      uint32_t *cnt = d_gcnt + (1 + g) * CC_SIZE;
      cd.cnt = cnt;
      cd.cand = d_cand + sb.o_cand; cd.cap_cand = sb.cap_cand;
      cd.bias_raw = d_bias + 2 * sb.o_cand; cd.vit_fast = d_vfast + sb.o_cand; cd.vit_exact = d_vexact + sb.o_cand; cd.vit_flag = d_vflag + sb.o_cand; cd.route = d_route + sb.o_cand;
      cd.vq = d_vq + sb.o_vq; cd.vxq = d_vxq + sb.o_vq; cd.cap_vq = sb.cap_cand;
      cd.fq = d_fq + sb.o_f; cd.bq = d_bq + sb.o_f; cd.cap_fq = sb.cap_f;
      cd.eq = d_eq + sb.o_e; cd.cap_eq = sb.cap_e;
      cd.rq = d_rq + sb.o_r; cd.cap_rq = sb.cap_r;
      cd.ensq = d_ensq + (size_t)ens_slot(part) * cp.rwork; cd.ensq_cnt = d_gcnt + CC_ENSQ + ens_slot(part);
      PairRec *nores = d_nores + sb.o_nores;
      const SsvEpi epi{lt, cd.cand, cnt + CC_CAND, sb.cap_cand, nores, cnt + CC_NORES, sb.cap_nores, nullptr};
      if (launch_ssv(sb.Q, (int)sb.nblocks, ssv_threads_for(sb.Q), sv, ctx->work.as<SsvBlockWork>() + sb.first, dm, res, off, dlen,
                     s->d_order.as<uint32_t>(), epi))
        throw Error(CKM_ERANGE, "no SSV kernel instance for this model length");
      st.ssv_launches++;
      hipStream_t sc = sv;
      if (NCH > 0) { sc = ctx->side[NSS + gi_now % NCH]; HIPCHK(hipEventRecord(ctx->grp_ev[g], sv)); HIPCHK(hipStreamWaitEvent(sc, ctx->grp_ev[g], 0)); }
      if (stop >= 2) {
        const WorkQueue qn{nullptr, cnt + CC_NORES, sb.cap_nores};
        if (sb.Q == kSsvNone) launch_msv_full(sc, GRID_MSV, qn, nores, dm, lt, res, off, dlen, nullptr, nullptr, std::max(64, sb.maxM), &cd);
        else if (launch_msv16(sb.Q >= 100 ? (sb.Q - 100 + 1) / 2 : sb.Q, GRID_MSV, sc, qn, nores, dm, lt, res, off, dlen, cd)) throw Error(CKM_ERANGE, "no exact-MSV kernel instance for this model length");
      }
      if (stop >= 3) launch_bias_filter(sc, GRID_MSV, cd, dm, lt, res, off);
      int rc = 0;
      for (int c = NVC - 1; c >= 0; --c) if (sb.vit[c] && stop >= 4) {
        const WorkQueue qv{cd.vq + (size_t)c * cd.cap_vq, cnt + CC_VQ + c, cd.cap_vq};
        if (c < NV16) rc |= launch_vit16(kVit16Q[c], GRID_VIT, sc, qv, cd.cand, dm, lt, res, off, dlen, cd);
        else rc |= launch_vit(kVitQH[c - NV16], GRID_VIT, sc, qv, cd.cand, dm, lt, res, off, dlen, nullptr, nullptr, nullptr, true, &cd);
      }
      for (int c = NVC - 1; c >= NV16; --c) if (sb.vit[c] && stop >= 5)
        rc |= launch_vit(kVitQH[c - NV16], std::max(64u, GRID_VIT / 4), sc, WorkQueue{cd.vxq + (size_t)c * cd.cap_vq, cnt + CC_VXQ + c, cd.cap_vq}, cd.cand, dm, lt, res, off, dlen, nullptr, nullptr, nullptr, false, &cd);
      for (int c = NFC - 1; c >= 0; --c) if (sb.fb[c]) {
        const int Q = kFbQ[c];
        const WorkQueue qf{cd.fq + (size_t)c * sb.cap_f, cnt + CC_FQ + c, sb.cap_f}, qb{cd.bq + (size_t)c * sb.cap_f, cnt + CC_BQ + c, sb.cap_f};
        const WorkQueue qe{cd.eq + (size_t)c * sb.cap_e, cnt + CC_EQ + c, sb.cap_e}, qr{cd.rq + (size_t)c * sb.cap_r, cnt + CC_RQ + c, sb.cap_r};
        if (stop >= 6) rc |= launch_fwd(Q, GRID_FB, sc, qf, cd.fwork, dm, lt, res, off, ws, d_fout_f, d_events_f, d_gcnt + CC_EVENTS, cp.events_f, &cd);
        if (stop >= 7) rc |= launch_bwd(Q, GRID_FB, sc, qb, cd.fwork, dm, lt, res, off, ws, d_fout_f, nullptr);
        if (stop >= 8) launch_regions(sc, 1024, qb.list, qb.count, sb.cap_f, cd.fwork, cd, dm, ws);
        if (stop >= 9) rc |= launch_fwd(Q, GRID_FB, sc, qe, cd.ework, dm, lt, res, off, ws, d_fout_e, d_events_e, d_gcnt + CC_EVENTS_E, cp.events_e, nullptr);
        if (stop >= 10) rc |= launch_bwd(Q, GRID_FB, sc, qe, cd.ework, dm, lt, res, off, ws, d_fout_e, d_rerr_e);
        if (stop >= 11) rc |= launch_oa(Q, GRID_FB, sc, qe, cd.ework, dm, ws, d_rerr_e, d_fout_e, d_envout);
        if (stop >= 12) rc |= launch_fwd(Q, std::max(64u, GRID_FB / 8), sc, qr, cd.rwork, dm, lt, res, off, ws, d_fout_r, d_events_r, d_gcnt + CC_EVENTS_R, 1 << 16, nullptr);
      }
      if (rc) throw Error(CKM_ERANGE, "no kernel instance for this model length");
    }
    if (cur_part >= 0) flush_part(cur_part);
    if (ens_launched) HIPCHK(hipEventRecord(ctx->ens_ev[16], es));
    ctx->ens_pending = ens_launched;
  }
  for (int k = 0; k < NSS; ++k) { HIPCHK(hipEventRecord(ctx->cls_ev[k], ctx->side[k])); HIPCHK(hipStreamWaitEvent(ms, ctx->cls_ev[k], 0)); }
  HIPCHK(hipEventRecord(ctx->ev[1], ms));
  HIPCHK(hipEventRecord(ctx->cev[1], ms));
  for (int k = NSS; k < NS; ++k) HIPCHK(hipEventRecord(ctx->cls_ev[k], ctx->side[k]));
  if (baton_lock.owns_lock()) { baton.k ^= 1; HIPCHK(hipEventRecord(baton.ev[baton.k], ms)); baton.recorded = true; baton_lock.unlock(); }
  {
    std::unique_lock<std::mutex> lock(owner->ssv_mutex);
    owner->ssv_prev_done = ctx->cev[1];
    took_turn = true; owner->ssv_turn++; owner->ssv_cv.notify_all();
  }
  hipStream_t drain = ctx->ens_stream;
  for (int k = NSS; k < NS; ++k) HIPCHK(hipStreamWaitEvent(drain, ctx->cls_ev[k], 0));
  HIPCHK(hipStreamWaitEvent(drain, ctx->cev[1], 0));
  ctx->ens_pending = false;
  HIPCHK(hipMemcpyAsync(h_cnt, d_gcnt, (NG + 1) * CC_SIZE * sizeof(uint32_t), hipMemcpyDeviceToHost, drain));
  unsigned long long *h_tops = pin_table<unsigned long long>(ctx->h_tops, 4);
  HIPCHK(hipMemcpyAsync(h_tops, d_tops, 4 * sizeof(unsigned long long), hipMemcpyDeviceToHost, drain));
  HIPCHK(hipGetLastError());
  CKM_TRACE_PT("chain queued");
  HIPCHK(hipStreamSynchronize(drain));
  CKM_TRACE_PT("chain drained");
  if (stop < 99) {
    fprintf(stderr, "ckm-chain w%d stop=%d:", ctx->id, stop);
    for (int k = 0; k < CC_END; ++k) { uint64_t v = h_cnt[k]; for (size_t g = 0; g < NG; ++g) v += h_cnt[(1 + g) * CC_SIZE + k]; if (v) fprintf(stderr, " c%d=%llu", k, (unsigned long long)v); }
    fprintf(stderr, "\n");
    return 1;
  }
  { float msv = 0.f; HIPCHK(hipEventElapsedTime(&msv, ctx->ev[0], ctx->ev[1])); st.ms_ssv = msv; }
  const double t_host0 = now_ms();
  st.ms_filters = t_host0 - t_start;

  const uint32_t n_fwork = h_cnt[CC_FWORK], n_ework = h_cnt[CC_EWORK], n_rwork = h_cnt[CC_RWORK],
                 n_pass = h_cnt[CC_PASS], n_reg = h_cnt[CC_REG], n_evf = h_cnt[CC_EVENTS], n_eve = h_cnt[CC_EVENTS_E], status = h_cnt[CC_STATUS];
  bool fits = status == 0;
  const bool tr = getenv("CKM_TRACE") != nullptr;
  auto over = [&](const char *what, int g, int k, uint64_t n, uint64_t cap) {
    fits = false; if (tr) fprintf(stderr, "ckm-trace w%d table %s (group %d, class %d) wanted %llu of %llu\n", ctx->id, what, g, k, (unsigned long long)n, (unsigned long long)cap); };
  auto need = [&](const char *what, uint32_t &cap, uint32_t n) { if (n > cap) { over(what, -1, -1, n, cap); cap = (uint32_t)std::min<uint64_t>((uint64_t)n + n / 4 + 1024, 0xfffffff0ull); } };
  cp.seen_rwork = std::max(cp.seen_rwork, n_rwork);
  need("fwork", cp.fwork, n_fwork); need("ework", cp.ework, n_ework); need("rwork", cp.rwork, n_rwork); need("pass", cp.pass, n_pass);
  need("reg", cp.reg, n_reg); need("events_f", cp.events_f, n_evf); need("events_e", cp.events_e, n_eve);
  uint32_t halved = 0;
  auto learn = [&](int kind, uint32_t &div, uint32_t &floor_, uint64_t pairs, uint64_t want) {
    const uint64_t w = want + want / 4 + 16;
    if ((pairs / std::max<uint64_t>(1, (uint64_t)div * shrink) >= floor_ || shrink > 1) && !((halved >> kind) & 1u)) { div = std::max<uint32_t>(1, div / 2); halved |= 1u << kind; }
    if (shrink == 1) floor_ = (uint32_t)std::min<uint64_t>(std::max<uint64_t>(floor_, w), 1u << 14);
    if (shrink == 1 && w > (1u << 14)) {
      const uint64_t d = pairs / w;
      if (d >= 1) div = (uint32_t)std::min<uint64_t>(div, d);
      else { div = 1; floor_ = (uint32_t)std::min<uint64_t>(std::max<uint64_t>(floor_, w), 1u << 20); }
    }
  };
  uint64_t n_cand = 0, n_nores = 0;
  for (size_t g = 0; g < NG; ++g) {
    const uint32_t *c = h_cnt + (1 + g) * CC_SIZE; const Sub &sb = subs[g];
    n_cand += c[CC_CAND]; n_nores += c[CC_NORES];
    if (c[CC_CAND] > sb.cap_cand) { over("cand", (int)g, -1, c[CC_CAND], sb.cap_cand); learn(0, cp.div_cand, cp.fl_cand, sb.pairs, c[CC_CAND]); }
    if (c[CC_NORES] > sb.cap_nores) { over("nores", (int)g, -1, c[CC_NORES], sb.cap_nores); if (sb.Q != kSsvNone) learn(1, cp.div_nores, cp.fl_nores, sb.pairs, c[CC_NORES]); }
    for (int k = 0; k < NVC; ++k) {
      st.pairs_vit += c[CC_VQ + k]; st.pairs_vit_exact += c[CC_VXQ + k];
      const uint32_t v = std::max(c[CC_VQ + k], c[CC_VXQ + k]);
      if (v > sb.cap_cand) { over("vq", (int)g, k, v, sb.cap_cand); learn(0, cp.div_cand, cp.fl_cand, sb.pairs, v); }
    }
    for (int k = 0; k < NFC; ++k) {
      const uint32_t f = std::max(c[CC_FQ + k], c[CC_BQ + k]);
      if (f > sb.cap_f) { over("fq", (int)g, k, f, sb.cap_f); learn(2, cp.div_fwork, cp.fl_fwork, sb.pairs, f); }
      if (c[CC_EQ + k] > sb.cap_e) { over("eq", (int)g, k, c[CC_EQ + k], sb.cap_e); learn(3, cp.div_ework, cp.fl_ework, sb.pairs, c[CC_EQ + k]); }
      if (c[CC_RQ + k] > sb.cap_r) { over("rq", (int)g, k, c[CC_RQ + k], sb.cap_r); learn(4, cp.div_rwork, cp.fl_rwork, sb.pairs, c[CC_RQ + k]); }
    }
  }
  if (status & CS_RWORK) cp.hens *= 2;
  st.ws_cap_bytes = ctx->ws.cap; st.ws_used_bytes = (std::min<uint64_t>(h_tops[0], cd0.ws_cap) + h_tops[2]) * 4;
  if (h_tops[0] > cd0.ws_cap && tr && cd0.ws_cap == ((ws_floats / 2) & ~(uint64_t)31))
    fprintf(stderr, "ckm-trace w%d workspace zone 1 is held to half of the workspace (%.3f GB) and this search asked for %.3f GB: it stays on the host-driven cascade\n", ctx->id,
            (double)cd0.ws_cap * 4 / 1e9, (double)h_tops[0] * 4 / 1e9);
  if (h_tops[0] > cd0.ws_cap) cp.z1_per_pair = std::max(cp.z1_per_pair, (float)(1.15 * (double)h_tops[0] * 4.0 / (double)std::max<uint64_t>(total_pairs, 1)));
  if (h_tops[2] > cd0.ws2_cap)
    cp.ws_per_cell = std::max(cp.ws_per_cell, (float)(1.15 * (double)(h_tops[2] + cd0.ws_cap) * 4.0 / std::max(cell_sum, 1.0)));
  if (tr) fprintf(stderr, "ckm-trace w%d workspace: %.3f GB held, %.3f GB asked for by this search (zone 1 %.3f of %.3f, zone 2 %.3f of %.3f), %.3e cells -> %.2f B per cell (estimate %.2f)\n", ctx->id,
                  (double)ctx->ws.cap / 1e9, (double)(h_tops[0] + h_tops[2]) * 4 / 1e9, (double)h_tops[0] * 4 / 1e9, (double)cd0.ws_cap * 4 / 1e9, (double)h_tops[2] * 4 / 1e9,
                  (double)cd0.ws2_cap * 4 / 1e9, cell_sum, (double)(h_tops[0] + h_tops[2]) * 4 / std::max(cell_sum, 1.0), (double)cp.ws_per_cell);
  if (!fits) {
    if (getenv("CKM_TRACE")) fprintf(stderr, "ckm-trace w%d device cascade did not fit (status 0x%x): host-driven cascade for this lane\n", ctx->id, status);
    return 1;
  }
  st.pairs_msv_full = n_nores; st.pairs_bias = n_cand; st.pairs_fwd = n_fwork; st.pairs_dom = n_pass; st.regions_multi = n_rwork;
  const CascadeDev &cd = cd0;

  const uint64_t n_hens = std::min<uint64_t>(h_tops[1], cp.hens);
  PassRec *h_pass = pin_table<PassRec>(ctx->h_pass, n_pass);
  RegionRec *h_reg = pin_table<RegionRec>(ctx->h_reg, n_reg);
  EnvOut *h_envout = pin_table<EnvOut>(ctx->h_envout, n_ework);
  ScaleEvent *h_events_f = pin_table<ScaleEvent>(ctx->h_events_f, n_evf), *h_events_e = pin_table<ScaleEvent>(ctx->h_events_e, n_eve);
  float *h_hens = pin_table<float>(ctx->h_hens, n_hens);
  hipStream_t rs = ctx->late[0];
  if (n_pass) HIPCHK(hipMemcpyAsync(h_pass, cd.h_pass, (size_t)n_pass * sizeof(PassRec), hipMemcpyDeviceToHost, rs));
  if (n_reg) HIPCHK(hipMemcpyAsync(h_reg, cd.h_reg, (size_t)n_reg * sizeof(RegionRec), hipMemcpyDeviceToHost, rs));
  if (n_ework) HIPCHK(hipMemcpyAsync(h_envout, d_envout, (size_t)n_ework * sizeof(EnvOut), hipMemcpyDeviceToHost, rs));
  if (n_evf) HIPCHK(hipMemcpyAsync(h_events_f, d_events_f, (size_t)n_evf * sizeof(ScaleEvent), hipMemcpyDeviceToHost, rs));
  if (n_eve) HIPCHK(hipMemcpyAsync(h_events_e, d_events_e, (size_t)n_eve * sizeof(ScaleEvent), hipMemcpyDeviceToHost, rs));
  if (n_hens) HIPCHK(hipMemcpyAsync(h_hens, d_hens, (size_t)n_hens * sizeof(float), hipMemcpyDeviceToHost, rs));
  HIPCHK(hipStreamSynchronize(rs));
  CKM_TRACE_PT("results copied");
  const PassRec *pass = h_pass;
  const RegionRec *reg = h_reg;
  std::vector<RegionRes> pre(n_reg);
  std::vector<uint8_t> pre_overflow(n_reg, 0);
  {
    std::vector<uint32_t> multi_rec;
    for (uint32_t ro = 0; ro < n_reg; ++ro) {
      const RegionRec &rr = reg[ro];
      if (!rr.multi || rr.pass >= n_pass) continue;
      if (rr.target == 0xffffffffu || (rr.target != REGION_DEFERRED && rr.pad == 0xffffffffu)) return 1;
      if (rr.target != REGION_DEFERRED) multi_rec.push_back(ro);
    }
    pool_run(ctx, multi_rec.size(), 1, [&](size_t lo, size_t hi) {
      for (size_t k = lo; k < hi; ++k) {
        const uint32_t ro = multi_rec[k];
        const RegionRec &rr = reg[ro]; RegionRes &o = pre[ro];
        const int Ld = rr.j - rr.i + 1, cap = std::min(Ld, 16);
        const float *raw = h_hens + rr.pad;
        const int32_t *ns = reinterpret_cast<const int32_t *>(raw);
        const int32_t *sg = reinterpret_cast<const int32_t *>(raw + 256);
        bool overflow = false;
        for (int t = 0; t < ENS_NSAMPLES; ++t) overflow |= ns[t] < 0;
        if (overflow) { pre_overflow[ro] = 1; continue; }
        o.cap = cap; o.nseg.assign(ns, ns + ENS_NSAMPLES); o.segs.assign((size_t)ENS_NSAMPLES * cap, Seg{0, 0, 0, 0});
        for (int t = 0; t < ENS_NSAMPLES; ++t)
          for (int d = 0; d < ns[t]; ++d) {
            const int32_t *q4 = sg + ((size_t)t * cap + (ns[t] - 1 - d)) * 4;
            o.segs[(size_t)t * cap + d] = Seg{q4[0], q4[1], q4[2], q4[3]};
          }
        const float *n2 = raw + 256 + (size_t)ENS_NSAMPLES * cap * 4;
        o.n2sum.assign(n2, n2 + Ld);
        cluster_ensemble(o);
      }
    });
  }
  std::vector<EnvReq> early_req; std::vector<EnvRes> early_res;
  std::vector<int64_t> early_first(n_reg, -1);
  for (uint32_t ro = 0; ro < n_reg; ++ro) {
    if (pre[ro].nseg.empty()) continue;
    const RegionRec &rr = reg[ro];
    early_first[ro] = (int64_t)early_req.size();
    for (const Seg &e : pre[ro].env) early_req.push_back({pass[rr.pass].model, pass[rr.pass].seq, e.sqfrom + rr.i - 1, e.sqto + rr.i - 1});
  }
  if (getenv("CKM_TRACE")) {
    size_t nm = 0, nl = 0;
    for (uint32_t ro = 0; ro < n_reg; ++ro) if (reg[ro].multi && reg[ro].pass < n_pass) { ++nm; nl += s->len[pass[reg[ro].pass].seq] > Lcut; }
    fprintf(stderr, "ckm-trace w%d %zu multi-domain regions, %zu of them on sequences of the long part (L > %d); %zu ensemble envelopes\n", ctx->id, nm, nl, Lcut, early_req.size());
  }
  CKM_TRACE_PT("clustering done");
  std::exception_ptr early_err;
  struct LateGuard { Worker *w; ~LateGuard() { w->late_round = false; } } late_guard{ctx};
  ctx->late_round = late_on() && baton.searches.load() > 1;
  std::thread early_thread;
  if (!early_req.empty())
    early_thread = std::thread([&] {
      try { HIPCHK(hipSetDevice(ctx->device)); rescore_envelopes(ctx, p, s, early_req, early_res); } catch (...) { early_err = std::current_exception(); }
    });
  struct Joiner { std::thread &t; ~Joiner() { if (t.joinable()) t.join(); } } early_joiner{early_thread};

  EventIndex fev; fev.build(h_events_f, n_evf, n_fwork);
  EventIndex eev; eev.build(h_events_e, n_eve, n_ework);
  std::vector<uint8_t> alive(n_pass, 0); std::vector<float> fwdsc(n_pass, 0.f);
  std::atomic<int> inconsistent{0};
  pool_run(ctx, n_pass, 256, [&](size_t lo, size_t hi) {
    for (size_t k = lo; k < hi; ++k) {
      const PassRec &r = pass[k];
      const HostProfile &hp = p->prof[r.model];
      const int L = s->len[r.seq];
      const LenEntry &le = s->lentab[L];
      const float p1 = (float)L / (float)(L + 1);
      const float nullb = (float)(log((double)r.bias_d) + (double)r.bias_e * kLn2);
      const float filtersc = nullb + (float)L * logf(p1) + logf(1.0f - p1);
      const float sc = bits(r.usc, filtersc);
      if (!(sc >= hp.thr_msv_f1)) continue;
      if (!(sc >= hp.thr_msv_f2)) {
        const uint32_t route = r.route & 0x0fu;
        if (route == 0) { inconsistent++; continue; }
        if (route == 1) {
          if (!(bits(r.vit_fast, filtersc) >= hp.thr_vit_f2)) { if (r.vit_flag) inconsistent++; continue; }
        } else if (!(bits(r.vit_exact, filtersc) >= hp.thr_vit_f2)) continue;
      }
      const float f = finish_forward(r.fwd_xC, le.move_m, fev.scales(r.fwork));
      if (!(bits(f, filtersc) >= hp.thr_fwd_f3)) continue;
      alive[k] = 1; fwdsc[k] = f;
    }
  });
  if (inconsistent.load()) throw Error(CKM_EHIP, "device-side filter decision contradicts the exact one (margin too small): please report");

  std::vector<uint32_t> rorder(n_reg);
  std::iota(rorder.begin(), rorder.end(), 0u);
  std::sort(rorder.begin(), rorder.end(), [&](uint32_t a, uint32_t b) { return reg[a].pass != reg[b].pass ? reg[a].pass < reg[b].pass : reg[a].i < reg[b].i; });
  DomStage ds;
  std::vector<int32_t> dsidx(n_pass, -1);
  for (uint32_t k = 0; k < n_pass; ++k) if (alive[k]) { dsidx[k] = (int32_t)ds.pass.size(); ds.pass.push_back({pass[k].model, pass[k].seq, fwdsc[k]}); }
  ds.nregions.assign(ds.pass.size(), 0);
  ds.env_of_pass.assign(ds.pass.size(), {0, 0});
  std::vector<RegionReq> redo_req; std::vector<size_t> redo_at;
  size_t n_deferred = 0;
  std::vector<uint32_t> item_rec;
  for (uint32_t ro : rorder) {
    const RegionRec &rr = reg[ro];
    if (rr.pass >= n_pass || dsidx[rr.pass] < 0) continue;
    const uint32_t q = (uint32_t)dsidx[rr.pass];
    if (rr.target == 0xffffffffu) return 1;
    ds.nregions[q]++;
    item_rec.push_back(ro);
    if (!rr.multi) { ds.items.push_back({q, rr.i, rr.j, -1}); continue; }
    ds.items.push_back({q, rr.i, rr.j, (int)ds.regres.size()});
    if (rr.target == REGION_DEFERRED || pre_overflow[ro]) {
      redo_req.push_back({pass[rr.pass].model, pass[rr.pass].seq, rr.i, rr.j}); redo_at.push_back(ds.regres.size());
      if (rr.target == REGION_DEFERRED) ++n_deferred;
      ds.regres.emplace_back();
    } else ds.regres.push_back(std::move(pre[ro]));
  }
  std::vector<int64_t> env_src;
  auto list_envelopes = [&]() {
    ds.envreq.clear(); ds.env_region.clear(); env_src.clear();
    size_t it = 0;
    for (size_t q = 0; q < ds.pass.size(); ++q) {
      ds.env_of_pass[q].first = ds.envreq.size();
// ... 260 lines not shown
```

checkm_amd/csrc/dev_types.h:

```cpp
#pragma once
#include <cstdint>

namespace ckm {

struct DevModel {
  int32_t M, ssvQ, fbQ, vitQH;
  int32_t fb_cls, vit_cls;
  int32_t vitx_cls, vit16Q;
  int32_t base_b, bias_b, tbm_b, tec_b;
  float   scale_b;
  float   scale_w; int32_t base_w, wE_loop, wE_move;
  float   fE_loop, fE_move;
  float   bt00, bt01, bt10, bt11, bpi0, bpi1;
  float   beo1[30];
  float   thr_msv_f1, thr_msv_f2, thr_vit_f2, thr_fwd_f3;
  float   thr_msv_f1_nat;
  const int16_t *ssv_tbl;
  const uint16_t *ssv_tbl_h;
  const uint16_t *ssv8_tbl_h;
  const uint8_t *rbv;
  const uint32_t *vit_e;
  const uint32_t *vit_t;
  const uint32_t *vit16_e;
  const uint32_t *vit16_t;
  const float   *rf;
  const float   *ftr;
};

constexpr int SSV_GROUP_BYTES = 30 * 256;
constexpr int SSV8_TWO_MAX_Q = 16;
constexpr bool ssv8_two_alignments_class(int Q8) { return Q8 >= 1 && Q8 <= SSV8_TWO_MAX_Q; }
constexpr bool ssv8_two_alignments(int M, int Q8) { return ssv8_two_alignments_class(Q8) && M < 16 * Q8; }
constexpr int ssv8_odd_base(int Q8) { return (Q8 + 3) / 4 * SSV_GROUP_BYTES; }
constexpr int ssv8_lds_bytes(int Q8) { return (ssv8_two_alignments_class(Q8) ? ssv8_odd_base(Q8) : 0) + (Q8 + 3) / 4 * SSV_GROUP_BYTES; }

struct LenEntry {
  float   loop_m, move_m;
  float   loop_u, move_u;
  float   nullsc;
  float   bias_tail;
  int32_t w_move;
  int32_t tjb_b;
};

struct SsvBlockWork {
  uint32_t model;
  uint32_t list_start;
  uint32_t count;
  uint32_t pair_start;
};

struct PairRec {
  uint32_t model, seq;
  float    usc;
  float    filtersc;
};

struct ScaleEvent {
  uint32_t slot; int32_t row; float scale; uint32_t pad;
};

struct FwdOut {
  float xC; int32_t nscale;
};

constexpr uint64_t FB_PATH_WITH_PP = 1ull << 63;
struct FbWork {
  uint32_t model, seq;
  int32_t  i0, Ld, Lcfg, multihit;
  uint64_t xs_off;
  uint64_t aux_off;
  uint64_t mxf_off, mxb_off;
  uint64_t path_off;
  uint32_t slot, full;
  uint32_t cand, pass;
};

struct WorkQueue { const uint32_t *list; const uint32_t *count; uint32_t cap; };

constexpr int ENS_NSAMPLES = 200;

struct EnsWork {
  uint32_t model, seq;
  int32_t  i0, Ld, Lcfg, cap;
  uint64_t xs_off, mx_off;
  uint64_t code_off;
  uint64_t ratio_off;
  uint64_t seg_off, nseg_off;
  uint64_t n2_off;
  uint64_t host_off;
};

struct SsvEpi {
  const LenEntry *lentab;
  PairRec *survivors; uint32_t *nsurv; uint32_t cap_surv;
  PairRec *noresult;  uint32_t *nnores; uint32_t cap_nores;
  uint16_t *maxv;
};

constexpr int NV16 = 12;
constexpr int NVW = 14;
constexpr int NVC = NV16 + NVW;
constexpr int NFC = 12;

enum CascadeCounter : int {
  CC_CAND = 0, CC_NORES, CC_FWORK, CC_EWORK, CC_RWORK, CC_PASS, CC_REG, CC_EVENTS, CC_STATUS, CC_EVENTS_E, CC_EVENTS_R,
  CC_ENSQ = 11,
  CC_VQ = 16, CC_VXQ = CC_VQ + NVC, CC_FQ = CC_VXQ + NVC, CC_BQ = CC_FQ + NFC, CC_EQ = CC_BQ + NFC, CC_RQ = CC_EQ + NFC, CC_END = CC_RQ + NFC
};
constexpr int CC_SIZE = 128;
static_assert(CC_END <= CC_SIZE, "counter block too small");

enum CascadeStatus : uint32_t {
  CS_CAND = 1, CS_VQ = 2, CS_FWORK = 4, CS_EWORK = 8, CS_RWORK = 16, CS_PASS = 32, CS_REG = 64, CS_EVENTS = 128,
  CS_WS = 256
};

struct PassRec {
  uint32_t cand, fwork, model, seq;
  float    usc, bias_d, bias_e;
  float    vit_fast, vit_exact;
  uint32_t vit_flag, route;
  float    fwd_xC; int32_t nscale;
};

constexpr uint32_t REGION_DEFERRED = 0xfffffffeu;

struct RegionRec {
  uint32_t pass; int32_t i, j;
  int32_t  multi;
  uint32_t target;
  uint32_t pad;
};

struct CascadeDev {
  PairRec *cand; uint32_t cap_cand;
  float *bias_raw;
  float *vit_fast, *vit_exact; uint32_t *vit_flag; uint8_t *route;
  uint32_t *vq, *vxq; uint32_t cap_vq;
  uint32_t *fq, *bq, *eq, *rq; uint32_t cap_fq, cap_eq, cap_rq;
  uint32_t *cnt;
  uint32_t *gcnt;
  FbWork *fwork; uint32_t cap_fwork;
  FbWork *ework; uint32_t cap_ework;
  FbWork *rwork; EnsWork *ens; uint32_t cap_rwork;
  uint32_t *ensq; uint32_t *ensq_cnt;
  unsigned long long *ws_top; unsigned long long ws_cap;
  unsigned long long *ws2_top; unsigned long long ws2_base, ws2_cap;
  PassRec *h_pass; uint32_t cap_pass;
  RegionRec *h_reg; uint32_t cap_reg;
  unsigned long long *hens_top; unsigned long long hens_cap;
  const int32_t *seq_len;
  float margin_msv, margin_vit, margin_fwd;
  uint32_t env_inplace;
};

struct EnvOut {
  float   xC; int32_t nscale;
  float   oasc;
  int32_t hmm_from, hmm_to, ali_from, ali_to;
  int32_t range_err;
  float   null2[20];
};

}
```

checkm_amd/csrc/kernels_fb.hip:

```cpp
#include <hip/hip_runtime.h>
#include <cstring>
#include "dev_types.h"
#include "cascade_dev.h"
#include "cascade_regions.h"
#include "xlane.h"

namespace ckm {



constexpr float NEGINF_F = -__builtin_inff();

template <int Q>
__device__ __forceinline__ int lds_cell(int c) { return (c % Q) * 64 + c / Q; }

template <int Q>
struct Tr {
  const float *t; int lane;
  __device__ __forceinline__ float BM(int q) const { return t[0 * Q * 64 + q * 64 + lane]; }
  __device__ __forceinline__ float MM(int q) const { return t[1 * Q * 64 + q * 64 + lane]; }
  __device__ __forceinline__ float IM(int q) const { return t[2 * Q * 64 + q * 64 + lane]; }
  __device__ __forceinline__ float DM(int q) const { return t[3 * Q * 64 + q * 64 + lane]; }
  __device__ __forceinline__ float MI(int q) const { return t[4 * Q * 64 + q * 64 + lane]; }
  __device__ __forceinline__ float II(int q) const { return t[5 * Q * 64 + q * 64 + lane]; }
// ... 20 lines not shown
  __syncthreads();
}

template <int Q>
__device__ __forceinline__ float fwd_row(float (&Mv)[Q], float (&Iv)[Q], float (&Dv)[Q], const Tr<Q> &tr,
                                         const float (&rfx)[Q], float xB, int lane) {
  const float mpi = lane_up1(Mv[Q - 1], 0.f), ipi = lane_up1(Iv[Q - 1], 0.f), dpi = lane_up1(Dv[Q - 1], 0.f);
  float Mn[Q], In[Q], Dn[Q], md[Q];
#pragma unroll
  for (int q = 0; q < Q; ++q) {
    const float mp = q ? Mv[q - 1] : mpi, ip = q ? Iv[q - 1] : ipi, dp = q ? Dv[q - 1] : dpi;
    float sv = xB * tr.BM(q);
    sv = sv + mp * tr.MM(q);
    sv = sv + ip * tr.IM(q);
    sv = sv + dp * tr.DM(q);
    Mn[q] = sv * rfx[q];
    const float a = Mv[q] * tr.MI(q), b = Iv[q] * tr.II(q);
    In[q] = a + b;
    md[q] = Mn[q] * tr.MD(q);
  }
  float a = 1.0f, b = 0.0f;
#pragma unroll
  for (int q = 0; q < Q; ++q) { const float dd = tr.DD(q); const float t = dd * b; b = md[q] + t; a = dd * a; }
  scan_up(a, b, lane);
  float d = lane_up1(b, 0.0f);
#pragma unroll
  for (int q = 0; q < Q; ++q) { Dn[q] = d; const float t = tr.DD(q) * d; d = md[q] + t; }
  float s = 0.f;
#pragma unroll
  for (int q = 0; q < Q; ++q) { s = s + Mn[q]; s = s + Dn[q]; }
  s = wave_sum(s);
#pragma unroll
  for (int q = 0; q < Q; ++q) { Mv[q] = Mn[q]; Iv[q] = In[q]; Dv[q] = Dn[q]; }
  return s;
}

template <int Q>
__device__ __forceinline__ void fwd_item(const FbWork &w, const DevModel &md, float *lds, int lane, const LenEntry *__restrict__ lentab,
                                         const uint8_t *__restrict__ res, const uint64_t *__restrict__ seq_off, float *__restrict__ ws,
                                         ScaleEvent *__restrict__ events, uint32_t *__restrict__ nevents, uint32_t cap_events,
                                         float &o_xC, int &o_nscale, float &o_lsum, float &o_move) {
  constexpr int Mp = Q * 64;
  Tr<Q> tr{lds, lane};
  const uint8_t *rp = res + seq_off[w.seq] + w.i0;
  const LenEntry le = lentab[w.Lcfg];
  const float loop = w.multihit ? le.loop_m : le.loop_u, move = w.multihit ? le.move_m : le.move_u;
  const float Eloop = w.multihit ? md.fE_loop : 0.0f, Emove = w.multihit ? md.fE_move : 1.0f;
  float Mv[Q], Iv[Q], Dv[Q];
#pragma unroll
  for (int q = 0; q < Q; ++q) Mv[q] = Iv[q] = Dv[q] = 0.f;
  float xN = 1.0f, xB = xN * move, xE = 0.f, xJ = 0.f, xC = 0.f;
  int nscale = 0;
  float lsum = 0.f;
  float *xs = ws + w.xs_off;
  float *mx = w.full ? ws + w.mxf_off : nullptr;
  if (lane == 0) { xs[0] = 0.f; xs[1] = xN; xs[2] = 0.f; xs[3] = xB; xs[4] = 0.f; xs[5] = 1.0f; }
  if (mx) {
    if (w.full == 2) {
      float4 *r4 = reinterpret_cast<float4 *>(mx) + lane * Q;
#pragma unroll
      for (int q = 0; q < Q; ++q) r4[q] = make_float4(0.f, 0.f, 0.f, 0.f);
    } else {
#pragma unroll
      for (int q = 0; q < Q; ++q) { mx[q * 64 + lane] = 0.f; mx[Mp + q * 64 + lane] = 0.f; }
    }
  }
  const gp<float> rf = gptr(md.rf);
  ResUp feed; feed.init(rp, w.Ld, lane);
  float rfc[Q];
  {
    const gp<float> r0 = rf + (size_t)feed.get(0) * Mp + lane;
#pragma unroll
    for (int q = 0; q < Q; ++q) rfc[q] = r0[q * 64];
  }
  for (int i = 1; i <= w.Ld; ++i) {
    float rfn[Q];
    {
      const int xn = feed.get((i < w.Ld) ? i : i - 1);
      const gp<float> r1 = rf + (size_t)xn * Mp + lane;
#pragma unroll
      for (int q = 0; q < Q; ++q) rfn[q] = r1[q * 64];
    }
    xE = fwd_row<Q>(Mv, Iv, Dv, tr, rfc, xB, lane);
#pragma unroll
    for (int q = 0; q < Q; ++q) rfc[q] = rfn[q];
    xN = xN * loop;
    { const float a = xC * loop, b = xE * Emove; xC = a + b; }
    { const float a = xJ * loop, b = xE * Eloop; xJ = a + b; }
    { const float a = xJ * move, b = xN * move; xB = a + b; }
    float scale = 1.0f;
    if (xE > 1.0e4f) {
      const float inv = 1.0f / xE;
      xN = xN / xE; xC = xC / xE; xJ = xJ / xE; xB = xB / xE;
#pragma unroll
      for (int q = 0; q < Q; ++q) { Mv[q] *= inv; Iv[q] *= inv; Dv[q] *= inv; }
      scale = xE; xE = 1.0f; ++nscale;
      lsum += approx_ln(scale);
      if (lane == 0) {
        const uint32_t e = atomicAdd(nevents, 1u);
        if (e < cap_events) { ScaleEvent ev; ev.slot = w.slot; ev.row = i; ev.scale = scale; ev.pad = 0; events[e] = ev; }
      }
    }
    if (lane == 0) { float *r = xs + (size_t)i * 6; r[0] = xE; r[1] = xN; r[2] = xJ; r[3] = xB; r[4] = xC; r[5] = scale; }
    if (mx) {
      if (w.full == 2) {
        float4 *r4 = reinterpret_cast<float4 *>(mx) + (size_t)i * Mp + lane * Q;
#pragma unroll
        for (int q = 0; q < Q; ++q) r4[q] = make_float4(Mv[q], Iv[q], Dv[q], 0.f);
      } else {
        float *r = mx + (size_t)i * 3 * Mp + lane;
#pragma unroll
        for (int q = 0; q < Q; ++q) { r[q * 64] = Mv[q]; r[Mp + q * 64] = Iv[q]; }
      }
    }
  }
  o_xC = xC; o_nscale = nscale; o_lsum = lsum; o_move = move;
}

template <int Q>
__global__ void __launch_bounds__(64) fwd_kernel(WorkQueue queue, FbWork *__restrict__ work,
                                                const DevModel *__restrict__ models, const LenEntry *__restrict__ lentab,
                                                const uint8_t *__restrict__ res, const uint64_t *__restrict__ seq_off,
                                                float *__restrict__ ws, FwdOut *__restrict__ out,
                                                ScaleEvent *__restrict__ events, uint32_t *__restrict__ nevents, uint32_t cap_events,
                                                CascadeDev cd, int decide) {
  extern __shared__ __attribute__((aligned(16))) float lds[];
  const int lane = threadIdx.x;
  uint32_t cur_model = 0xffffffffu;
 const uint32_t nqueue = queue_len(queue);
 for (uint32_t qk = blockIdx.x; qk < nqueue; qk += gridDim.x) {
  const uint32_t item = queue.list[qk];
  const FbWork w = work[item];
  const DevModel &md = models[w.model];
  if (w.model != cur_model) { load_tr<Q>(lds, md.ftr); cur_model = w.model; }
  float xC, lsum, move; int nscale;
  fwd_item<Q>(w, md, lds, lane, lentab, res, seq_off, ws, events, nevents, cap_events, xC, nscale, lsum, move);
  if (lane == 0) { out[w.slot].xC = xC; out[w.slot].nscale = nscale; }
  if (decide && lane == 0) {
    const PairRec pr = cd.cand[w.cand];
    const float fwdsc = lsum + approx_ln(xC * move);
    const float sc = (fwdsc - pr.filtersc) * LOG2E_F;
    if (sc >= md.thr_fwd_f3 - cd.margin_fwd) {
      unsigned long long off;
      if (ws_alloc(cd, (unsigned long long)(w.Ld + 1) * 3ull, off)) {
        const uint32_t pid = atomicAdd(&cd.gcnt[CC_PASS], 1u);
        if (pid < cd.cap_pass) {
          PassRec r;
          r.cand = w.cand; r.fwork = item; r.model = w.model; r.seq = w.seq; r.usc = pr.usc;
          r.bias_d = cd.bias_raw[2 * (size_t)w.cand]; r.bias_e = cd.bias_raw[2 * (size_t)w.cand + 1];
          r.vit_fast = cd.vit_fast[w.cand]; r.vit_exact = cd.vit_exact[w.cand]; r.vit_flag = cd.vit_flag[w.cand]; r.route = cd.route[w.cand];
          r.fwd_xC = xC; r.nscale = nscale;
          cd.h_pass[pid] = r;
          work[item].aux_off = off; work[item].pass = pid;
          queue_push(cd, cd.bq, CC_BQ, md.fb_cls, cd.cap_fq, item, (uint32_t)CS_FWORK);
        } else atomicOr(&cd.gcnt[CC_STATUS], (uint32_t)CS_PASS);
      }
    }
  }
 }
}

#define CKM_LD2(p) __hip_atomic_load((p), __ATOMIC_RELAXED, __HIP_MEMORY_SCOPE_AGENT)
template <int Q>
__device__ __forceinline__ void bwd_dchain(float (&Dn)[Q], const float (&av)[Q], const Tr<Q> &tr, int lane) {
  float a = 1.0f, b = 0.0f;
#pragma unroll
  for (int q = Q - 1; q >= 0; --q) { const float dd = tr.DD(q); const float t = dd * b; b = av[q] + t; a = dd * a; }
  scan_down(a, b, lane);
  float d = lane_down1(b, 0.0f);
#pragma unroll
  for (int q = Q - 1; q >= 0; --q) { const float t = tr.DD(q) * d; d = av[q] + t; Dn[q] = d; }
}

template <int Q, bool XL>
__device__ __forceinline__ void bwd_item(const FbWork &w, const DevModel &md, float *lds, int lane, const LenEntry *__restrict__ lentab,
                                         const uint8_t *__restrict__ res, const uint64_t *__restrict__ seq_off, float *__restrict__ ws,
                                         float fwd_xC, bool &o_bad) {
  constexpr int Mp = Q * 64;
  Tr<Q> tr{lds, lane};
  const uint8_t *rp = res + seq_off[w.seq] + w.i0;
  const LenEntry le = lentab[w.Lcfg];
  const float loop = w.multihit ? le.loop_m : le.loop_u, move = w.multihit ? le.move_m : le.move_u;
  const float Eloop = w.multihit ? md.fE_loop : 0.0f, Emove = w.multihit ? md.fE_move : 1.0f;
  const float *xs = ws + w.xs_off;
  float *aux = ws + w.aux_off;
  const float *fm = w.full ? ws + w.mxf_off : nullptr;
  float *bm = w.full ? ws + w.mxb_off : nullptr;
  const size_t pst = (w.mxb_off == w.mxf_off) ? (size_t)3 * Mp : (size_t)2 * Mp;
  const int L = w.Ld;
  const float invZ = 1.0f / (fwd_xC * move);
  float tIMn[Q], tMMn[Q], tDMn[Q];
#pragma unroll
  for (int q = 0; q < Q; ++q) {
    const int c = lane * Q + q + 1;
    tMMn[q] = (c < Mp) ? tr.at(1, c) : 0.f; tIMn[q] = (c < Mp) ? tr.at(2, c) : 0.f; tDMn[q] = (c < Mp) ? tr.at(3, c) : 0.f;
  }
  float Mv[Q], Iv[Q], Dv[Q];
  float xC = move, xE = xC * Emove, xJ = 0.f, xB = 0.f, xN = 0.f;
  {
    float av[Q];
#pragma unroll
    for (int q = 0; q < Q; ++q) av[q] = xE + 0.0f;
    bwd_dchain<Q>(Dv, av, tr, lane);
    const float dnx = lane_down1(Dv[0], 0.f);
#pragma unroll
    for (int q = 0; q < Q; ++q) {
      const float dn1 = (q + 1 < Q) ? Dv[q + 1] : dnx;
      float m = xE + 0.0f; m = m + 0.0f; m = m + tr.MD(q) * dn1;
      Mv[q] = m; Iv[q] = 0.f;
    }
  }
  bool bad = false;
  float fMr[Q], fIr[Q];
  auto fetch_f = [&](int r) {
    if (w.full && r >= 1) {
      const float *__restrict__ f = fm + (size_t)r * 3 * Mp + lane;
#pragma unroll
      for (int q = 0; q < Q; ++q) { fMr[q] = f[q * 64]; fIr[q] = f[Mp + q * 64]; }
    }
  };
  fetch_f(L);
  float rowU[6], rowC[6], rowD[6];
  auto load_row = [&](float (&dst)[6], int r) {
    const float *x = xs + (size_t)(r < 0 ? 0 : r) * 6;
#pragma unroll
    for (int k = 0; k < 6; ++k) dst[k] = XL ? CKM_LD2(&x[k]) : x[k];
  };
  load_row(rowC, L); load_row(rowD, L - 1);
#pragma unroll
  for (int k = 0; k < 6; ++k) rowU[k] = 1.0f;
  auto emit = [&](int r) {
    if (w.full) {
      if (r >= 1) {
        float *__restrict__ b = bm + (size_t)r * pst + lane;
        float pmv[Q], piv[Q];
#pragma unroll
        for (int q = 0; q < Q; ++q) {
          float pm = fMr[q] * Mv[q]; pm = pm * invZ;
          float pi = fIr[q] * Iv[q]; pi = pi * invZ;
          pmv[q] = pm; piv[q] = pi;
          if (!(__builtin_isfinite(pm) && __builtin_isfinite(pi))) bad = true;
        }
        fetch_f(r - 1);
#pragma unroll
        for (int q = 0; q < Q; ++q) { b[q * 64] = pmv[q]; b[Mp + q * 64] = piv[q]; }
        if (lane == 0) {
          const float wgt = invZ / rowC[5];
          float t;
          t = rowD[1] * xN; t = t * loop; aux[(size_t)r * 3 + 0] = t * wgt;
          t = rowD[2] * xJ; t = t * loop; aux[(size_t)r * 3 + 1] = t * wgt;
          t = rowD[4] * xC; t = t * loop; aux[(size_t)r * 3 + 2] = t * wgt;
        }
      }
    } else if (lane == 0) {
      if (r >= 1) {
        float et = rowC[0] * xE; et = et * invZ;
        const float wgt = invZ / rowC[5];
        float a = rowD[1] * xN; a = a * loop;
        float b = rowD[2] * xJ; b = b * loop;
        float c = rowD[4] * xC; c = c * loop;
        aux[(size_t)r * 3 + 1] = et;
        aux[(size_t)r * 3 + 2] = ((a + b) + c) * wgt;
      }
      if (r < L) { float bt = rowC[3] * xB; bt = bt * invZ; aux[(size_t)(r + 1) * 3 + 0] = bt; }
    }
  };
  emit(L);
  const gp<float> rf = gptr(md.rf);
  ResDown feed; feed.init(rp, max(L, 1), lane);
  float rfc[Q];
  if (L >= 1) {
    const gp<float> r0 = rf + (size_t)feed.get(L - 1) * Mp + lane;
#pragma unroll
    for (int q = 0; q < Q; ++q) rfc[q] = r0[q * 64];
  }
  for (int i = L - 1; i >= 0; --i) {
#pragma unroll
    for (int k = 0; k < 6; ++k) { rowU[k] = rowC[k]; rowC[k] = rowD[k]; }
    load_row(rowD, i - 1);
    float rfn[Q];
    {
      const int xn = feed.get((i >= 1) ? i - 1 : 0);
      const gp<float> r1 = rf + (size_t)xn * Mp + lane;
#pragma unroll
      for (int q = 0; q < Q; ++q) rfn[q] = r1[q * 64];
    }
    float mn[Q];
#pragma unroll
    for (int q = 0; q < Q; ++q) mn[q] = Mv[q] * rfc[q];
#pragma unroll
    for (int q = 0; q < Q; ++q) rfc[q] = rfn[q];
    float s = 0.f;
#pragma unroll
    for (int q = 0; q < Q; ++q) { const float t = tr.BM(q) * mn[q]; s = s + t; }
    xB = wave_sum(s);
    { const float a = xB * move, b = xJ * loop; xJ = a + b; }
    xC = xC * loop;
    { const float a = xC * Emove, b = xJ * Eloop; xE = a + b; }
    { const float a = xB * move, b = xN * loop; xN = a + b; }
    const float mnx = lane_down1(mn[0], 0.f);
    float av[Q];
#pragma unroll
    for (int q = 0; q < Q; ++q) { const float mn1 = (q + 1 < Q) ? mn[q + 1] : mnx; av[q] = xE + tDMn[q] * mn1; }
    float Dn[Q];
    bwd_dchain<Q>(Dn, av, tr, lane);
    const float dnx = lane_down1(Dn[0], 0.f);
    float Mn[Q], In[Q];
// ... 276 lines not shown
```

Baseline: 288,100.

## Batch Forward/Backward queues across consecutive groups sharing a float class

Groups within a part that share a Forward/Backward class now push into one shared queue per batch instead of per-group queues. The float stages (fwd, bwd, regions, envelope, OA) are launched once per batch after its last group, with cross-stream event waits on the earlier groups. This cuts the number of small float kernel launches and gives each launch more work per grid. The cost is a longer dependency chain before the float stages start, extra queue-routing logic in the push path, and new capacity-learning code per batch.

Result: no change. 290,900, median of 6 (+1.0%).

```diff
diff --git a/checkm_amd/csrc/cascade_dev.h b/checkm_amd/csrc/cascade_dev.h
--- a/checkm_amd/csrc/cascade_dev.h
+++ b/checkm_amd/csrc/cascade_dev.h
@@ -30,6 +30,18 @@
   if (pos < cap) lists[(size_t)cls * cap + pos] = value; else atomicOr(&cd.gcnt[CC_STATUS], overflow_bit);
 }
 
+template <int COUNTER>
+__device__ __forceinline__ void float_push(const CascadeDev &cd, int cls, uint32_t value, uint32_t overflow_bit) {
+  const bool alt = cd.alt_cls1 == (uint32_t)cls + 1u;
+  uint32_t *lists = COUNTER == CC_FQ ? (alt ? cd.alt_fq : cd.fq) : COUNTER == CC_BQ ? (alt ? cd.alt_bq : cd.bq)
+                  : COUNTER == CC_EQ ? (alt ? cd.alt_eq : cd.eq) : (alt ? cd.alt_rq : cd.rq);
+  const uint32_t cap = (COUNTER == CC_FQ || COUNTER == CC_BQ) ? (alt ? cd.alt_cap_fq : cd.cap_fq)
+                     : COUNTER == CC_EQ ? (alt ? cd.alt_cap_eq : cd.cap_eq) : (alt ? cd.alt_cap_rq : cd.cap_rq);
+  uint32_t *cnt = alt ? cd.alt_fcnt : cd.fcnt;
+  const uint32_t pos = atomicAdd(&cnt[COUNTER + cls], 1u);
+  if (pos < cap) lists[((alt || cd.fq_one) ? (size_t)0 : (size_t)cls * cap) + pos] = value; else atomicOr(&cd.gcnt[CC_STATUS], overflow_bit);
+}
+
 __device__ __forceinline__ void pass_to_forward(const CascadeDev &cd, const DevModel &md, uint32_t pi, uint32_t model, uint32_t seq) {
   const int L = cd.seq_len[seq];
   unsigned long long off;
@@ -39,9 +51,9 @@
   FbWork w;
   w.model = model; w.seq = seq; w.i0 = 0; w.Ld = L; w.Lcfg = L; w.multihit = 1;
   w.xs_off = off; w.aux_off = 0; w.mxf_off = 0; w.mxb_off = 0; w.path_off = 0;
-  w.slot = t; w.full = 0; w.cand = pi; w.pass = 0xffffffffu;
+  w.slot = t; w.full = 0; w.cand = cd.cand_base + pi; w.pass = 0xffffffffu;
   cd.fwork[t] = w;
-  queue_push(cd, cd.fq, CC_FQ, md.fb_cls, cd.cap_fq, t, (uint32_t)CS_FWORK);
+  float_push<CC_FQ>(cd, md.fb_cls, t, (uint32_t)CS_FWORK);
 }
 
 }
diff --git a/checkm_amd/csrc/cascade_regions.h b/checkm_amd/csrc/cascade_regions.h
--- a/checkm_amd/csrc/cascade_regions.h
+++ b/checkm_amd/csrc/cascade_regions.h
@@ -37,7 +37,7 @@
         w.xs_off = off + xs; w.aux_off = off + aux; w.mxf_off = off + mf; w.mxb_off = off + mb; w.path_off = 0;
         w.slot = e; w.full = 1; w.cand = pw.cand; w.pass = pw.pass;
         cd.ework[e] = w;
-        queue_push(cd, cd.eq, CC_EQ, md.fb_cls, cd.cap_eq, e, (uint32_t)CS_EWORK);
+        float_push<CC_EQ>(cd, md.fb_cls, e, (uint32_t)CS_EWORK);
         rec.target = e;
       } else atomicOr(&cd.gcnt[CC_STATUS], (uint32_t)CS_EWORK);
     }
@@ -70,7 +70,7 @@
         w.xs_off = e.xs_off; w.aux_off = 0; w.mxf_off = e.mx_off; w.mxb_off = 0; w.path_off = 0;
         w.slot = r; w.full = 2; w.cand = pw.cand; w.pass = pw.pass;
         cd.rwork[r] = w;
-        queue_push(cd, cd.rq, CC_RQ, md.fb_cls, cd.cap_rq, r, (uint32_t)CS_RWORK);
+        float_push<CC_RQ>(cd, md.fb_cls, r, (uint32_t)CS_RWORK);
         if (cd.ensq) { const uint32_t k = atomicAdd(cd.ensq_cnt, 1u); if (k < cd.cap_rwork) cd.ensq[k] = r; }
         rec.target = r;
       } else atomicOr(&cd.gcnt[CC_STATUS], (uint32_t)CS_RWORK);
diff --git a/checkm_amd/csrc/ckm_api.hip b/checkm_amd/csrc/ckm_api.hip
--- a/checkm_amd/csrc/ckm_api.hip
+++ b/checkm_amd/csrc/ckm_api.hip
@@ -81,6 +81,7 @@
       for (auto &e : w.cev) HIPCHK(hipEventCreateWithFlags(&e, hipEventDisableTiming));
       for (auto &e : w.cls_ev) HIPCHK(hipEventCreateWithFlags(&e, hipEventDisableTiming));
       for (auto &e : w.grp_ev) HIPCHK(hipEventCreateWithFlags(&e, hipEventDisableTiming));
+      for (auto &e : w.chn_ev) HIPCHK(hipEventCreateWithFlags(&e, hipEventDisableTiming));
       for (auto &e : w.ens_ev) HIPCHK(hipEventCreateWithFlags(&e, hipEventDisableTiming));
       memset(&w.stats, 0, sizeof(w.stats));
       w.ws_budget = budget;
@@ -120,6 +121,7 @@
     for (auto &e : w.cev) if (e) (void)hipEventDestroy(e);
     for (auto &e : w.cls_ev) if (e) (void)hipEventDestroy(e);
     for (auto &e : w.grp_ev) if (e) (void)hipEventDestroy(e);
+    for (auto &e : w.chn_ev) if (e) (void)hipEventDestroy(e);
     for (auto &e : w.ens_ev) if (e) (void)hipEventDestroy(e);
     if (w.late[0]) (void)hipStreamDestroy(w.late[0]);
     if (!w.own_streams) continue;
diff --git a/checkm_amd/csrc/ckm_debug.hip b/checkm_amd/csrc/ckm_debug.hip
--- a/checkm_amd/csrc/ckm_debug.hip
+++ b/checkm_amd/csrc/ckm_debug.hip
@@ -226,7 +226,7 @@
     cd.vq = (uint32_t *)table(ctx->c_vq, (size_t)n * NVC * 4); cd.vxq = (uint32_t *)table(ctx->c_vxq, (size_t)n * NVC * 4); cd.cap_vq = n;
     cd.fq = (uint32_t *)table(ctx->c_fq, (size_t)n * NFC * 4); cd.cap_fq = n;
     cd.fwork = (FbWork *)table(ctx->c_fwork, (size_t)n * sizeof(FbWork)); cd.cap_fwork = n;
-    cd.gcnt = d_cnt; cd.cnt = d_cnt + CC_SIZE;
+    cd.gcnt = d_cnt; cd.cnt = d_cnt + CC_SIZE; cd.fcnt = cd.cnt;
     cd.ws_top = d_tops; cd.ws_cap = 2 * ws_need;
     cd.seq_len = dlen;
     cd.margin_msv = kMarginMsv; cd.margin_vit = kMarginVit; cd.margin_fwd = kMarginFwd;
diff --git a/checkm_amd/csrc/ckm_host.h b/checkm_amd/csrc/ckm_host.h
--- a/checkm_amd/csrc/ckm_host.h
+++ b/checkm_amd/csrc/ckm_host.h
@@ -18,6 +18,7 @@
 #include "dev_types.h"
 #include "host_pool.h"
 #include "stream_plan.h"
+#include "float_batches.h"
 
 namespace ckm {
 
@@ -262,6 +263,7 @@
   hipStream_t late[4] = {};
   bool late_round = false;
   hipEvent_t grp_ev[192] = {};
+  hipEvent_t chn_ev[192] = {};
 };
 
 constexpr int kVitQH[ckm::NVW] = {1, 2, 3, 4, 5, 6, 7, 8, 10, 12, 14, 16, 24, 32};
diff --git a/checkm_amd/csrc/ckm_search.hip b/checkm_amd/csrc/ckm_search.hip
--- a/checkm_amd/csrc/ckm_search.hip
+++ b/checkm_amd/csrc/ckm_search.hip
@@ -586,7 +586,7 @@
     }
   }
   struct Sub { int Q; int maxM = 0; size_t first, nblocks; uint64_t pairs = 0; bool vit[NVC] = {false}, fb[NFC] = {false};
-               uint32_t cap_cand = 0, cap_nores = 0, cap_f = 0, cap_e = 0, cap_r = 0; size_t o_cand = 0, o_nores = 0, o_vq = 0, o_f = 0, o_e = 0, o_r = 0; };
+               uint32_t cap_cand = 0, cap_nores = 0, cap_f = 0, cap_e = 0, cap_r = 0; size_t o_cand = 0, o_nores = 0, o_vq = 0; };
   std::vector<Sub> subs;
   {
     std::map<int, size_t> at;
@@ -619,8 +619,34 @@
     sb.cap_r = capof(sb.pairs, cp.div_rwork, cp.fl_rwork);
     sb.o_cand = tot_cand; tot_cand += sb.cap_cand; sb.o_nores = tot_nores; tot_nores += sb.cap_nores;
     sb.o_vq = sb.o_cand * NVC;
-    sb.o_f = tot_f * NFC; tot_f += sb.cap_f; sb.o_e = tot_e * NFC; tot_e += sb.cap_e; sb.o_r = tot_r * NFC; tot_r += sb.cap_r;
-  }
+    tot_f += sb.cap_f; tot_e += sb.cap_e; tot_r += sb.cap_r;
+  }
+  if (tot_cand > 0xfffffff0ull) return 2;
+  std::vector<size_t> launch_order;
+  {
+    size_t g0 = 0;
+    for (int part = 0; part < nparts; ++part) {
+      size_t g1 = g0;
+      while (g1 < NG && groups[g1].first / 1000 == part) ++g1;
+      for (size_t g = g1; g-- > g0;) launch_order.push_back(g);
+      g0 = g1;
+    }
+  }
+  static_assert(kFloatClasses == NFC, "float_batches.h and dev_types.h disagree about the Forward/Backward classes");
+  FloatBatchPlan fbp;
+  {
+    std::vector<FloatGroup> fg;
+    for (size_t g : launch_order) {
+      const Sub &sb = subs[g];
+      FloatGroup x; x.part = groups[g].first / 1000; x.ssv_cls = sb.Q; x.pairs = sb.pairs; x.cap_f = sb.cap_f; x.cap_e = sb.cap_e; x.cap_r = sb.cap_r;
+      int ncls = 0;
+      for (int c = 0; c < NFC; ++c) if (sb.fb[c]) { x.fb_mask |= 1u << c; ++ncls; }
+      if (ncls > 2) return 2;
+      fg.push_back(x);
+    }
+    fbp = float_batch_plan(fg);
+  }
+  const size_t NB = fbp.batches.size();
   auto grow = [](uint32_t &v, uint64_t want) { if (v < want) v = (uint32_t)std::min<uint64_t>(want, 0xfffffff0ull); };
   grow(cp.fwork, tot_f); grow(cp.ework, tot_e); grow(cp.rwork, tot_r);
   grow(cp.pass, std::max<uint64_t>(1 << 13, tot_e)); grow(cp.reg, (uint64_t)cp.ework + cp.rwork);
@@ -636,15 +662,15 @@
   }
   const uint64_t ws_floats = ctx->ws.cap / 4;
   CKM_TRACE_PT("workspace ready");
-  uint32_t *d_gcnt = dev_table<uint32_t>(ctx->c_cnt, (NG + 1) * CC_SIZE);
+  uint32_t *d_gcnt = dev_table<uint32_t>(ctx->c_cnt, (NG + 1 + NB) * CC_SIZE);
   unsigned long long *d_tops = dev_table<unsigned long long>(ctx->c_tops, 4);
   CascadeDev cd0; memset(&cd0, 0, sizeof(cd0));
   PairRec *d_cand = dev_table<PairRec>(ctx->c_cand, tot_cand), *d_nores = dev_table<PairRec>(ctx->c_nores, tot_nores);
   float *d_bias = dev_table<float>(ctx->c_bias, tot_cand * 2), *d_vfast = dev_table<float>(ctx->c_vfast, tot_cand), *d_vexact = dev_table<float>(ctx->c_vexact, tot_cand);
   uint32_t *d_vflag = dev_table<uint32_t>(ctx->c_vflag, tot_cand); uint8_t *d_route = dev_table<uint8_t>(ctx->c_route, tot_cand);
   uint32_t *d_vq = dev_table<uint32_t>(ctx->c_vq, tot_cand * NVC), *d_vxq = dev_table<uint32_t>(ctx->c_vxq, tot_cand * NVC);
-  uint32_t *d_fq = dev_table<uint32_t>(ctx->c_fq, tot_f * NFC), *d_bq = dev_table<uint32_t>(ctx->c_bq, tot_f * NFC);
-  uint32_t *d_eq = dev_table<uint32_t>(ctx->c_eq, tot_e * NFC), *d_rq = dev_table<uint32_t>(ctx->c_rq, tot_r * NFC);
+  uint32_t *d_fq = dev_table<uint32_t>(ctx->c_fq, fbp.tot_f), *d_bq = dev_table<uint32_t>(ctx->c_bq, fbp.tot_f);
+  uint32_t *d_eq = dev_table<uint32_t>(ctx->c_eq, fbp.tot_e), *d_rq = dev_table<uint32_t>(ctx->c_rq, fbp.tot_r);
   cd0.gcnt = d_gcnt;
   cd0.fwork = dev_table<FbWork>(ctx->c_fwork, cp.fwork); cd0.cap_fwork = cp.fwork;
   cd0.ework = dev_table<FbWork>(ctx->c_ework, cp.ework); cd0.cap_ework = cp.ework;
@@ -667,7 +693,7 @@
   ScaleEvent *d_events_r = dev_table<ScaleEvent>(ctx->c_events_r, 1 << 16);
   EnvOut *d_envout = dev_table<EnvOut>(ctx->c_envout, cp.ework);
   ScaleEvent *d_events_f = dev_table<ScaleEvent>(ctx->c_events_f, cp.events_f), *d_events_e = dev_table<ScaleEvent>(ctx->c_events_e, cp.events_e);
-  uint32_t *h_cnt = pin_table<uint32_t>(ctx->h_cnt, (NG + 1) * CC_SIZE);
+  uint32_t *h_cnt = pin_table<uint32_t>(ctx->h_cnt, (NG + 1 + NB) * CC_SIZE);
   ensure_ens_seeds(ctx);
   float *ws = ctx->ws.as<float>();
   CKM_TRACE_PT("tables ready");
@@ -681,7 +707,7 @@
   }
   CKM_TRACE_PT("ssv turn taken");
   const int stop = getenv("CKM_CHAIN_STOP") ? atoi(getenv("CKM_CHAIN_STOP")) : 99;
-  HIPCHK(hipMemsetAsync(d_gcnt, 0, (NG + 1) * CC_SIZE * sizeof(uint32_t), ms));
+  HIPCHK(hipMemsetAsync(d_gcnt, 0, (NG + 1 + NB) * CC_SIZE * sizeof(uint32_t), ms));
   HIPCHK(hipMemsetAsync(d_tops, 0, 4 * sizeof(unsigned long long), ms));
   if (owner->ssv_prev_done) HIPCHK(hipStreamWaitEvent(ms, owner->ssv_prev_done, 0));
   DeviceBaton &baton = device_baton(owner->device);
@@ -695,17 +721,8 @@
   HIPCHK(hipEventRecord(ctx->ev[0], ms));
   HIPCHK(hipEventRecord(ctx->cev[0], ms));
   for (int k = 0; k < NS; ++k) HIPCHK(hipStreamWaitEvent(ctx->side[k], ctx->cev[0], 0));
-  {
-    std::vector<size_t> launch_order;
-    {
-      size_t g0 = 0;
-      for (int part = 0; part < nparts; ++part) {
-        size_t g1 = g0;
-        while (g1 < NG && groups[g1].first / 1000 == part) ++g1;
-        for (size_t g = g1; g-- > g0;) launch_order.push_back(g);
-        g0 = g1;
-      }
-    }
+  int float_launches = 0;
+  {
     int ens_Mp = NL;
     for (const Sub &sb : subs) for (int c = 0; c < NFC; ++c) if (sb.fb[c]) ens_Mp = std::max(ens_Mp, kFbQ[c] * NL);
     hipStream_t es = ctx->ens_stream;
@@ -720,6 +737,8 @@
       ens_launched = true;
     };
     int gi = 0, cur_part = -1;
+    size_t next_batch = 0;
+    auto chain_stream = [&](int pos) { return NCH > 0 ? ctx->side[NSS + pos % NCH] : ctx->side[pos % NSS]; };
     for (size_t g : launch_order) {
       const int gi_now = gi++;
       const Sub &sb = subs[g];
@@ -733,9 +752,21 @@
       cd.cand = d_cand + sb.o_cand; cd.cap_cand = sb.cap_cand;
       cd.bias_raw = d_bias + 2 * sb.o_cand; cd.vit_fast = d_vfast + sb.o_cand; cd.vit_exact = d_vexact + sb.o_cand; cd.vit_flag = d_vflag + sb.o_cand; cd.route = d_route + sb.o_cand;
       cd.vq = d_vq + sb.o_vq; cd.vxq = d_vxq + sb.o_vq; cd.cap_vq = sb.cap_cand;
-      cd.fq = d_fq + sb.o_f; cd.bq = d_bq + sb.o_f; cd.cap_fq = sb.cap_f;
-      cd.eq = d_eq + sb.o_e; cd.cap_eq = sb.cap_e;
-      cd.rq = d_rq + sb.o_r; cd.cap_rq = sb.cap_r;
+      cd.cand_base = (uint32_t)sb.o_cand;
+      cd.fq_one = 1;
+      for (int c = NFC - 1, k = 0; c >= 0; --c) if (sb.fb[c]) {
+        const int bi = fbp.batch_of(gi_now, c);
+        const FloatBatch &fb = fbp.batches[(size_t)bi];
+        uint32_t *bcnt = d_gcnt + (1 + NG + (size_t)bi) * CC_SIZE;
+        if (k++ == 0) {
+          cd.fq = d_fq + fb.o_f; cd.bq = d_bq + fb.o_f; cd.cap_fq = fb.cap_f; cd.eq = d_eq + fb.o_e; cd.cap_eq = fb.cap_e; cd.rq = d_rq + fb.o_r; cd.cap_rq = fb.cap_r;
+          cd.fcnt = bcnt;
+        } else {
+          cd.alt_cls1 = (uint32_t)c + 1u;
+          cd.alt_fq = d_fq + fb.o_f; cd.alt_bq = d_bq + fb.o_f; cd.alt_cap_fq = fb.cap_f; cd.alt_eq = d_eq + fb.o_e; cd.alt_cap_eq = fb.cap_e;
+          cd.alt_rq = d_rq + fb.o_r; cd.alt_cap_rq = fb.cap_r; cd.alt_fcnt = bcnt;
+        }
+      }
       cd.ensq = d_ensq + (size_t)ens_slot(part) * cp.rwork; cd.ensq_cnt = d_gcnt + CC_ENSQ + ens_slot(part);
       PairRec *nores = d_nores + sb.o_nores;
       const SsvEpi epi{lt, cd.cand, cnt + CC_CAND, sb.cap_cand, nores, cnt + CC_NORES, sb.cap_nores, nullptr};
@@ -759,13 +790,28 @@
       }
       for (int c = NVC - 1; c >= NV16; --c) if (sb.vit[c] && stop >= 5)
         rc |= launch_vit(kVitQH[c - NV16], std::max(64u, GRID_VIT / 4), sc, WorkQueue{cd.vxq + (size_t)c * cd.cap_vq, cnt + CC_VXQ + c, cd.cap_vq}, cd.cand, dm, lt, res, off, dlen, nullptr, nullptr, nullptr, false, &cd);
-      for (int c = NFC - 1; c >= 0; --c) if (sb.fb[c]) {
-        const int Q = kFbQ[c];
-        const WorkQueue qf{cd.fq + (size_t)c * sb.cap_f, cnt + CC_FQ + c, sb.cap_f}, qb{cd.bq + (size_t)c * sb.cap_f, cnt + CC_BQ + c, sb.cap_f};
-        const WorkQueue qe{cd.eq + (size_t)c * sb.cap_e, cnt + CC_EQ + c, sb.cap_e}, qr{cd.rq + (size_t)c * sb.cap_r, cnt + CC_RQ + c, sb.cap_r};
+      const size_t first_batch = next_batch;
+      while (next_batch < NB && fbp.batches[next_batch].issue_after == gi_now) ++next_batch;
+      bool waited_for = false;
+      for (size_t bi = next_batch; bi < NB && !waited_for; ++bi)
+        for (int m : fbp.batches[bi].waits) if (m == gi_now && chain_stream(fbp.batches[bi].issue_after) != sc) waited_for = true;
+      if (waited_for) HIPCHK(hipEventRecord(ctx->chn_ev[g], sc));
+      for (size_t bi = first_batch; bi < next_batch; ++bi) {
+        const FloatBatch &fb = fbp.batches[bi];
+        const int c = fb.cls, Q = kFbQ[c];
+        for (int m : fb.waits) if (chain_stream(m) != sc) HIPCHK(hipStreamWaitEvent(sc, ctx->chn_ev[launch_order[(size_t)m]], 0));
+        uint32_t *bcnt = d_gcnt + (1 + NG + bi) * CC_SIZE;
+        CascadeDev cd = cd0;
+        cd.cnt = bcnt; cd.fcnt = bcnt; cd.fq_one = 1;
+        cd.cand = d_cand; cd.bias_raw = d_bias; cd.vit_fast = d_vfast; cd.vit_exact = d_vexact; cd.vit_flag = d_vflag; cd.route = d_route;
+        cd.fq = d_fq + fb.o_f; cd.bq = d_bq + fb.o_f; cd.cap_fq = fb.cap_f; cd.eq = d_eq + fb.o_e; cd.cap_eq = fb.cap_e; cd.rq = d_rq + fb.o_r; cd.cap_rq = fb.cap_r;
+        cd.ensq = d_ensq + (size_t)ens_slot(part) * cp.rwork; cd.ensq_cnt = d_gcnt + CC_ENSQ + ens_slot(part);
+        const WorkQueue qf{cd.fq, bcnt + CC_FQ + c, fb.cap_f}, qb{cd.bq, bcnt + CC_BQ + c, fb.cap_f};
+        const WorkQueue qe{cd.eq, bcnt + CC_EQ + c, fb.cap_e}, qr{cd.rq, bcnt + CC_RQ + c, fb.cap_r};
+        float_launches += std::max(0, std::min(stop, 12) - 5);
         if (stop >= 6) rc |= launch_fwd(Q, GRID_FB, sc, qf, cd.fwork, dm, lt, res, off, ws, d_fout_f, d_events_f, d_gcnt + CC_EVENTS, cp.events_f, &cd);
         if (stop >= 7) rc |= launch_bwd(Q, GRID_FB, sc, qb, cd.fwork, dm, lt, res, off, ws, d_fout_f, nullptr);
-        if (stop >= 8) launch_regions(sc, 1024, qb.list, qb.count, sb.cap_f, cd.fwork, cd, dm, ws);
+        if (stop >= 8) launch_regions(sc, 1024, qb.list, qb.count, fb.cap_f, cd.fwork, cd, dm, ws);
         if (stop >= 9) rc |= launch_fwd(Q, GRID_FB, sc, qe, cd.ework, dm, lt, res, off, ws, d_fout_e, d_events_e, d_gcnt + CC_EVENTS_E, cp.events_e, nullptr);
         if (stop >= 10) rc |= launch_bwd(Q, GRID_FB, sc, qe, cd.ework, dm, lt, res, off, ws, d_fout_e, d_rerr_e);
         if (stop >= 11) rc |= launch_oa(Q, GRID_FB, sc, qe, cd.ework, dm, ws, d_rerr_e, d_fout_e, d_envout);
@@ -791,7 +837,7 @@
   for (int k = NSS; k < NS; ++k) HIPCHK(hipStreamWaitEvent(drain, ctx->cls_ev[k], 0));
   HIPCHK(hipStreamWaitEvent(drain, ctx->cev[1], 0));
   ctx->ens_pending = false;
-  HIPCHK(hipMemcpyAsync(h_cnt, d_gcnt, (NG + 1) * CC_SIZE * sizeof(uint32_t), hipMemcpyDeviceToHost, drain));
+  HIPCHK(hipMemcpyAsync(h_cnt, d_gcnt, (NG + 1 + NB) * CC_SIZE * sizeof(uint32_t), hipMemcpyDeviceToHost, drain));
   unsigned long long *h_tops = pin_table<unsigned long long>(ctx->h_tops, 4);
   HIPCHK(hipMemcpyAsync(h_tops, d_tops, 4 * sizeof(unsigned long long), hipMemcpyDeviceToHost, drain));
   HIPCHK(hipGetLastError());
@@ -800,7 +846,7 @@
   CKM_TRACE_PT("chain drained");
   if (stop < 99) {
     fprintf(stderr, "ckm-chain w%d stop=%d:", ctx->id, stop);
-    for (int k = 0; k < CC_END; ++k) { uint64_t v = h_cnt[k]; for (size_t g = 0; g < NG; ++g) v += h_cnt[(1 + g) * CC_SIZE + k]; if (v) fprintf(stderr, " c%d=%llu", k, (unsigned long long)v); }
+    for (int k = 0; k < CC_END; ++k) { uint64_t v = h_cnt[k]; for (size_t g = 0; g < NG + NB; ++g) v += h_cnt[(1 + g) * CC_SIZE + k]; if (v) fprintf(stderr, " c%d=%llu", k, (unsigned long long)v); }
     fprintf(stderr, "\n");
     return 1;
   }
@@ -812,8 +858,10 @@
                  n_pass = h_cnt[CC_PASS], n_reg = h_cnt[CC_REG], n_evf = h_cnt[CC_EVENTS], n_eve = h_cnt[CC_EVENTS_E], status = h_cnt[CC_STATUS];
   bool fits = status == 0;
   const bool tr = getenv("CKM_TRACE") != nullptr;
-  auto over = [&](const char *what, int g, int k, uint64_t n, uint64_t cap) {
-    fits = false; if (tr) fprintf(stderr, "ckm-trace w%d table %s (group %d, class %d) wanted %llu of %llu\n", ctx->id, what, g, k, (unsigned long long)n, (unsigned long long)cap); };
+  auto over_of = [&](const char *owner, const char *what, int g, int k, uint64_t n, uint64_t cap) {
+    fits = false; if (tr) fprintf(stderr, "ckm-trace w%d table %s (%s %d, class %d) wanted %llu of %llu\n", ctx->id, what, owner, g, k, (unsigned long long)n, (unsigned long long)cap); };
+  auto over = [&](const char *what, int g, int k, uint64_t n, uint64_t cap) { over_of("group", what, g, k, n, cap); };
+  auto over_batch = [&](const char *what, int b, int k, uint64_t n, uint64_t cap) { over_of("batch", what, b, k, n, cap); };
   auto need = [&](const char *what, uint32_t &cap, uint32_t n) { if (n > cap) { over(what, -1, -1, n, cap); cap = (uint32_t)std::min<uint64_t>((uint64_t)n + n / 4 + 1024, 0xfffffff0ull); } };
   cp.seen_rwork = std::max(cp.seen_rwork, n_rwork);
   need("fwork", cp.fwork, n_fwork); need("ework", cp.ework, n_ework); need("rwork", cp.rwork, n_rwork); need("pass", cp.pass, n_pass);
@@ -840,13 +888,21 @@
       const uint32_t v = std::max(c[CC_VQ + k], c[CC_VXQ + k]);
       if (v > sb.cap_cand) { over("vq", (int)g, k, v, sb.cap_cand); learn(0, cp.div_cand, cp.fl_cand, sb.pairs, v); }
     }
-    for (int k = 0; k < NFC; ++k) {
-      const uint32_t f = std::max(c[CC_FQ + k], c[CC_BQ + k]);
-      if (f > sb.cap_f) { over("fq", (int)g, k, f, sb.cap_f); learn(2, cp.div_fwork, cp.fl_fwork, sb.pairs, f); }
-      if (c[CC_EQ + k] > sb.cap_e) { over("eq", (int)g, k, c[CC_EQ + k], sb.cap_e); learn(3, cp.div_ework, cp.fl_ework, sb.pairs, c[CC_EQ + k]); }
-      if (c[CC_RQ + k] > sb.cap_r) { over("rq", (int)g, k, c[CC_RQ + k], sb.cap_r); learn(4, cp.div_rwork, cp.fl_rwork, sb.pairs, c[CC_RQ + k]); }
-    }
-  }
+  }
+  auto asked = [](uint32_t n, uint32_t total, uint32_t cap) { return total > cap && cap ? (uint32_t)std::min<uint64_t>(((uint64_t)n * total + cap - 1) / cap, 0xfffffff0ull) : n; };
+  uint32_t nonempty = 0;
+  for (size_t b = 0; b < NB; ++b) {
+    const uint32_t *c = h_cnt + (1 + NG + b) * CC_SIZE; const FloatBatch &fb = fbp.batches[b];
+    const int k = fb.cls;
+    const uint32_t f = std::max(asked(c[CC_FQ + k], n_fwork, cd0.cap_fwork), c[CC_BQ + k]);
+    const uint32_t e = asked(c[CC_EQ + k], n_ework, cd0.cap_ework), r = asked(c[CC_RQ + k], n_rwork, cd0.cap_rwork);
+    nonempty |= (c[CC_FQ + k] ? 1u : 0u) | (c[CC_BQ + k] ? 2u : 0u) | (c[CC_EQ + k] ? 4u : 0u) | (c[CC_RQ + k] ? 8u : 0u);
+    if (f > fb.cap_f) { over_batch("fq", (int)b, k, f, fb.cap_f); learn(2, cp.div_fwork, cp.fl_fwork, fb.pairs, f); }
+    if (e > fb.cap_e) { over_batch("eq", (int)b, k, e, fb.cap_e); learn(3, cp.div_ework, cp.fl_ework, fb.pairs, e); }
+    if (r > fb.cap_r) { over_batch("rq", (int)b, k, r, fb.cap_r); learn(4, cp.div_rwork, cp.fl_rwork, fb.pairs, r); }
+  }
+  if (tr) fprintf(stderr, "ckm-trace w%d float batches: %zu groups, %zu batches, %d float launches queued; queues with entries: fq %d bq %d eq %d rq %d\n", ctx->id,
+                  NG, NB, float_launches, (int)(nonempty & 1u), (int)((nonempty >> 1) & 1u), (int)((nonempty >> 2) & 1u), (int)((nonempty >> 3) & 1u));
   if (status & CS_RWORK) cp.hens *= 2;
   st.ws_cap_bytes = ctx->ws.cap; st.ws_used_bytes = (std::min<uint64_t>(h_tops[0], cd0.ws_cap) + h_tops[2]) * 4;
   if (h_tops[0] > cd0.ws_cap && tr && cd0.ws_cap == ((ws_floats / 2) & ~(uint64_t)31))
diff --git a/checkm_amd/csrc/dev_types.h b/checkm_amd/csrc/dev_types.h
--- a/checkm_amd/csrc/dev_types.h
+++ b/checkm_amd/csrc/dev_types.h
@@ -140,6 +140,11 @@
   uint32_t *vq, *vxq; uint32_t cap_vq;
   uint32_t *fq, *bq, *eq, *rq; uint32_t cap_fq, cap_eq, cap_rq;
   uint32_t *cnt;
+  uint32_t *fcnt;
+  uint32_t fq_one;
+  uint32_t alt_cls1;
+  uint32_t *alt_fq, *alt_bq, *alt_eq, *alt_rq, *alt_fcnt; uint32_t alt_cap_fq, alt_cap_eq, alt_cap_rq;
+  uint32_t cand_base;
   uint32_t *gcnt;
   FbWork *fwork; uint32_t cap_fwork;
   FbWork *ework; uint32_t cap_ework;
diff --git a/checkm_amd/csrc/float_batches.h b/checkm_amd/csrc/float_batches.h
--- /dev/null
+++ b/checkm_amd/csrc/float_batches.h
@@ -0,0 +1,65 @@
+#pragma once
+#include <algorithm>
+#include <cstdint>
+#include <vector>
+
+namespace ckm {
+
+constexpr int kFloatClasses = 12;
+constexpr uint64_t kFloatCapMax = 0x7ffffff0ull;
+
+struct FloatGroup {
+  int part = 0;
+  int ssv_cls = 0;
+  uint32_t fb_mask = 0;
+  uint64_t pairs = 0;
+  uint32_t cap_f = 0, cap_e = 0, cap_r = 0;
+};
+
+struct FloatBatch {
+  int part = 0, cls = 0;
+  int first = 0, count = 0;
+  int issue_after = 0;
+  std::vector<int> waits;
+  uint64_t pairs = 0;
+  uint32_t cap_f = 0, cap_e = 0, cap_r = 0;
+  uint64_t o_f = 0, o_e = 0, o_r = 0;
+};
+
+struct FloatBatchPlan {
+  std::vector<FloatBatch> batches;
+  std::vector<int> of;
+  uint64_t tot_f = 0, tot_e = 0, tot_r = 0;
+  int batch_of(int pos, int cls) const { return of[(size_t)pos * kFloatClasses + cls]; }
+};
+
+inline FloatBatchPlan float_batch_plan(const std::vector<FloatGroup> &groups) {
+  FloatBatchPlan p;
+  const int n = (int)groups.size();
+  p.of.assign((size_t)n * kFloatClasses, -1);
+  for (int pos = 0; pos < n; ++pos) {
+    for (int c = kFloatClasses - 1; c >= 0; --c) {
+      if (!((groups[pos].fb_mask >> c) & 1u)) continue;
+      const bool last = pos + 1 == n || groups[pos + 1].part != groups[pos].part || !((groups[pos + 1].fb_mask >> c) & 1u);
+      if (!last) continue;
+      FloatBatch b;
+      b.part = groups[pos].part; b.cls = c; b.issue_after = pos;
+      int first = pos;
+      while (first > 0 && groups[first - 1].part == b.part && ((groups[first - 1].fb_mask >> c) & 1u)) --first;
+      b.first = first; b.count = pos - first + 1;
+      uint64_t f = 0, e = 0, r = 0;
+      for (int k = first; k <= pos; ++k) {
+        const FloatGroup &g = groups[k];
+        if (k != pos) b.waits.push_back(k);
+        b.pairs += g.pairs; f += g.cap_f; e += g.cap_e; r += g.cap_r;
+        p.of[(size_t)k * kFloatClasses + c] = (int)p.batches.size();
+      }
+      b.cap_f = (uint32_t)std::min(f, kFloatCapMax); b.cap_e = (uint32_t)std::min(e, kFloatCapMax); b.cap_r = (uint32_t)std::min(r, kFloatCapMax);
+      b.o_f = p.tot_f; p.tot_f += b.cap_f; b.o_e = p.tot_e; p.tot_e += b.cap_e; b.o_r = p.tot_r; p.tot_r += b.cap_r;
+      p.batches.push_back(std::move(b));
+    }
+  }
+  return p;
+}
+
+}
diff --git a/checkm_amd/csrc/kernels_fb.hip b/checkm_amd/csrc/kernels_fb.hip
--- a/checkm_amd/csrc/kernels_fb.hip
+++ b/checkm_amd/csrc/kernels_fb.hip
@@ -196,7 +196,7 @@
           r.fwd_xC = xC; r.nscale = nscale;
           cd.h_pass[pid] = r;
           work[item].aux_off = off; work[item].pass = pid;
-          queue_push(cd, cd.bq, CC_BQ, md.fb_cls, cd.cap_fq, item, (uint32_t)CS_FWORK);
+          float_push<CC_BQ>(cd, md.fb_cls, item, (uint32_t)CS_FWORK);
         } else atomicOr(&cd.gcnt[CC_STATUS], (uint32_t)CS_PASS);
       }
     }
```
